# PABannier/bark.cpp

Measured on AMD Instinct MI355X. Metric: audio-sec/sec (RTF), bark-small f16 greedy, higher is better.
Workload: dtype f16 (f32 accumulate); 1 GPU; BASELINE config 2: bark-small f16 on 1xMI355X, single prompt per step, greedy, hipGraph decode, n_steps_text_encoder=256

## Files before the change

bark.cpp_amd/api.py:

```python
from __future__ import annotations

import ctypes as C
import math
import os
import subprocess

import numpy as np

_HERE = os.path.dirname(os.path.abspath(__file__))

PROGRESS_CB = C.CFUNCTYPE(None, C.c_void_p, C.c_int, C.c_int, C.c_void_p)


class BarkContextParams(C.Structure):
    _fields_ = [
        ("verbosity", C.c_int), ("temp", C.c_float), ("fine_temp", C.c_float), ("min_eos_p", C.c_float),
        ("sliding_window_size", C.c_int32), ("max_coarse_history", C.c_int32), ("sample_rate", C.c_int32),
        ("target_bandwidth", C.c_int32), ("cls_token_id", C.c_int32), ("sep_token_id", C.c_int32),
        ("n_steps_text_encoder", C.c_int32), ("text_pad_token", C.c_int32), ("text_encoding_offset", C.c_int32),
        ("semantic_rate_hz", C.c_float), ("semantic_pad_token", C.c_int32), ("semantic_vocab_size", C.c_int32),
        ("semantic_infer_token", C.c_int32), ("coarse_rate_hz", C.c_float), ("coarse_infer_token", C.c_int32),
        ("coarse_semantic_pad_token", C.c_int32), ("n_coarse_codebooks", C.c_int32), ("n_fine_codebooks", C.c_int32),
        ("codebook_size", C.c_int32), ("progress_callback", PROGRESS_CB), ("progress_callback_user_data", C.c_void_p),
    ]
# ... 9 lines not shown

class BarkHipVoicePrompt(C.Structure):
    _fields_ = [("semantic", C.c_void_p), ("n_semantic", C.c_int32), ("coarse_Tx2", C.c_void_p), ("n_coarse_frames", C.c_int32),
                ("fine_Tx8", C.c_void_p), ("n_fine_frames", C.c_int32)]


class BarkHipAudioFormat(C.Structure):
    _fields_ = [("sample_rate", C.c_int32), ("sample_format", C.c_int32)]


class BarkHipJoinParams(C.Structure):
    _fields_ = [("gap_samples", C.c_int32), ("fade_samples", C.c_int32), ("trim_threshold", C.c_float), ("trim_pad_frames", C.c_int32)]


class BarkHipLongParams(C.Structure):
    _fields_ = [("max_tokens", C.c_int32), ("chain", C.c_int32), ("join", BarkHipJoinParams)]


def join_params(gap_samples: int = 6000, fade_samples: int = 0, trim_threshold: float = 0.0, trim_pad_frames: int = 0) -> BarkHipJoinParams:
    return BarkHipJoinParams(int(gap_samples), int(fade_samples), float(trim_threshold), int(trim_pad_frames))


SPLIT_MAX_CHUNKS = 64
SAMPLE_F32, SAMPLE_S16, SAMPLE_MULAW = 0, 1, 2
SAMPLE_FORMATS = {"f32": SAMPLE_F32, "s16": SAMPLE_S16, "mulaw": SAMPLE_MULAW}
SAMPLE_DTYPES = {SAMPLE_F32: np.float32, SAMPLE_S16: np.int16, SAMPLE_MULAW: np.uint8}


def audio_format(rate: int = 24000, fmt="f32") -> BarkHipAudioFormat:
    return BarkHipAudioFormat(int(rate), SAMPLE_FORMATS[fmt] if isinstance(fmt, str) else int(fmt))


def speed_permille(speed) -> int:
    return int(math.floor(1000.0 * float(speed) + 0.5))


def _voice_struct(voice):
    sem = np.ascontiguousarray(voice.semantic, dtype=np.int32).reshape(-1)
    co = np.ascontiguousarray(voice.coarse, dtype=np.int32).reshape(-1, 2)
    fi = np.ascontiguousarray(voice.fine, dtype=np.int32).reshape(-1, 8)
    return BarkHipVoicePrompt(sem.ctypes.data, len(sem), co.ctypes.data, len(co), fi.ctypes.data, len(fi)), (sem, co, fi)


class BarkHipStats(C.Structure):
    _fields_ = [
        ("t_load_us", C.c_int64), ("t_eval_us", C.c_int64), ("t_semantic_us", C.c_int64), ("t_coarse_us", C.c_int64),
        ("t_fine_us", C.c_int64), ("t_codec_us", C.c_int64), ("n_sample_semantic", C.c_int64), ("n_sample_coarse", C.c_int64),
        ("n_sample_fine", C.c_int64), ("n_semantic", C.c_int32), ("n_frames", C.c_int32), ("n_samples", C.c_int32),
        ("n_near_tie", C.c_int32), ("graph_replays", C.c_int32), ("n_prefix_rows_reused", C.c_int32),
    ]

    def as_dict(self):
        return {k: getattr(self, k) for k, _ in self._fields_}


def library_path() -> str:
    return os.environ.get("BARK_HIP_LIBRARY") or os.path.join(_HERE, "lib", "libbark.so")


def build_library(force: bool = False) -> str:
    if force:
        subprocess.check_call(["rm", "-rf", os.path.join(_HERE, "lib", "obj")])
    subprocess.check_call([os.path.join(_HERE, "build.sh")])
    return library_path()


_LIB = None
VOICE_AUDIO_MAX_SAMPLES = 480000

EXPORTS = [
    "bark_context_default_params", "bark_load_model", "bark_generate_audio", "bark_get_audio_data", "bark_get_audio_data_size",
    "bark_get_load_time", "bark_get_eval_time", "bark_reset_statistics", "bark_model_quantize", "bark_free",
    "ggml_time_init", "ggml_time_us", "ggml_time_ms", "ggml_init", "ggml_free",
    "bark_hip_hparams", "bark_hip_set_params", "bark_hip_tokenize", "bark_hip_bert_tokenize", "bark_hip_gpt_eval",
    "bark_hip_fine_eval", "bark_hip_semantic", "bark_hip_coarse", "bark_hip_fine", "bark_hip_fine_many", "bark_hip_codec_decode", "bark_hip_codec_tap",
    "bark_hip_clone_context", "bark_hip_generate_audio_batch", "bark_hip_generate_batch", "bark_hip_generate_batch_seeded", "bark_hip_generate_batch_ex", "bark_hip_reserve_batch", "bark_hip_profile_lock_step", "bark_hip_batch_audio", "bark_hip_batch_tokens", "bark_hip_get_semantic_tokens", "bark_hip_get_coarse_tokens", "bark_hip_get_fine_tokens", "bark_hip_get_stats",
    "bark_hip_time_decode_step", "bark_hip_time_gemv", "bark_hip_time_slots", "bark_hip_time_fine_pass", "bark_hip_time_fine_passes", "bark_hip_describe", "bark_hip_set_fine_order", "bark_hip_load_model_on_device", "bark_hip_batcher_create_multi",
    "bark_hip_batcher_create", "bark_hip_batcher_create_ex", "bark_hip_batcher_submit", "bark_hip_batcher_submit_ex", "bark_hip_batcher_wait", "bark_hip_batcher_stats", "bark_hip_batcher_admitted", "bark_hip_batcher_free",
    "bark_hip_set_sampling_filter", "bark_hip_generate_batch_filtered", "bark_hip_batcher_submit_filtered", "bark_hip_sample_rows_filtered", "bark_hip_time_sample_filter",
    "bark_hip_set_voice_prompt", "bark_hip_generate_batch_voiced", "bark_hip_batcher_submit_voiced", "bark_hip_pick_rows",
    "bark_hip_has_codec_encoder", "bark_hip_codec_encode", "bark_hip_codec_encode_many", "bark_hip_codec_encode_tap", "bark_hip_rvq_encode", "bark_hip_codec_encode_latents", "bark_hip_codec_encode_device_us",
    "bark_hip_load_semantic_encoder", "bark_hip_has_semantic_encoder", "bark_hip_semantic_encode", "bark_hip_semantic_encode_tap", "bark_hip_semantic_head", "bark_hip_semantic_encode_device_us",
    "bark_hip_resample_taps", "bark_hip_resample_24k_to_16k", "bark_hip_voice_from_audio", "bark_hip_set_voice_from_audio", "bark_hip_time_resample",
    "bark_hip_batch_lock_steps",
    "bark_hip_resample_out_len", "bark_hip_resample_table", "bark_hip_resample", "bark_hip_resample_many", "bark_hip_get_audio_as", "bark_hip_batch_audio_as",
    "bark_hip_batcher_submit_as", "bark_hip_batcher_wait_bytes", "bark_hip_time_resample_pair",
    "bark_hip_split_text", "bark_hip_generate_long", "bark_hip_long_audio_as", "bark_hip_long_chunks", "bark_hip_long_chunk_audio", "bark_hip_long_chunk_tokens",
    "bark_hip_join_many", "bark_hip_time_join", "bark_hip_batcher_submit_long", "bark_hip_batcher_ticket_chunks", "bark_hip_time_join_activity",
    "bark_hip_tempo_out_len", "bark_hip_tempo_window", "bark_hip_tempo", "bark_hip_tempo_many", "bark_hip_tempo_positions", "bark_hip_get_audio_at",
    "bark_hip_batch_audio_at", "bark_hip_long_audio_at", "bark_hip_batcher_submit_at", "bark_hip_batcher_submit_long_at", "bark_hip_time_tempo",
]


def load_library() -> C.CDLL:
    global _LIB
    if _LIB is not None:
        return _LIB
    path = library_path()
    if not os.path.exists(path):
        raise RuntimeError(f"{path} is missing - run bark.cpp_amd/build.sh (there is no fallback path)")
    lib = C.CDLL(path)
    vp, ip, fp = C.c_void_p, C.c_void_p, C.c_void_p
    lib.bark_context_default_params.restype = BarkContextParams
    lib.bark_context_default_params.argtypes = []
    lib.bark_load_model.restype = vp
    lib.bark_load_model.argtypes = [C.c_char_p, BarkContextParams, C.c_uint32]
    lib.bark_generate_audio.restype = C.c_bool
    lib.bark_generate_audio.argtypes = [vp, C.c_char_p, C.c_int]
    lib.bark_get_audio_data.restype = C.POINTER(C.c_float)
    lib.bark_get_audio_data.argtypes = [vp]
    lib.bark_get_audio_data_size.restype = C.c_int
    lib.bark_get_audio_data_size.argtypes = [vp]
    lib.bark_get_load_time.restype = C.c_int64
    lib.bark_get_load_time.argtypes = [vp]
    lib.bark_get_eval_time.restype = C.c_int64
    lib.bark_get_eval_time.argtypes = [vp]
    lib.bark_reset_statistics.argtypes = [vp]
    lib.bark_model_quantize.restype = C.c_bool
    lib.bark_model_quantize.argtypes = [C.c_char_p, C.c_char_p, C.c_int]
    lib.bark_free.argtypes = [vp]
    lib.ggml_time_us.restype = C.c_int64
    lib.bark_hip_hparams.argtypes = [vp, C.c_int, ip]
    lib.bark_hip_set_params.argtypes = [vp, BarkContextParams]
    lib.bark_hip_tokenize.argtypes = [vp, C.c_char_p, ip]
    lib.bark_hip_bert_tokenize.argtypes = [vp, C.c_char_p, ip, C.c_int]
    lib.bark_hip_gpt_eval.argtypes = [vp, C.c_int, ip, C.c_int, C.c_int, C.c_int, fp]
    lib.bark_hip_fine_eval.argtypes = [vp, ip, C.c_int, fp]
    lib.bark_hip_semantic.argtypes = [vp, ip, ip, C.c_int, fp]
    lib.bark_hip_coarse.argtypes = [vp, ip, C.c_int, ip, C.c_int]
    lib.bark_hip_fine.argtypes = [vp, ip, C.c_int, ip, C.c_int]
    lib.bark_hip_fine_many.argtypes = [vp, ip, ip, C.c_int, ip, C.c_int]
    lib.bark_hip_codec_decode.argtypes = [vp, ip, C.c_int, C.c_int, fp, C.c_int]
    lib.bark_hip_codec_tap.argtypes = [vp, ip, C.c_int, C.c_int, C.c_int, fp, C.c_int]
    lib.bark_hip_has_codec_encoder.argtypes = [vp]
    lib.bark_hip_codec_encode.argtypes = [vp, fp, C.c_int, C.c_int, ip, C.c_int]
    lib.bark_hip_codec_encode_many.argtypes = [vp, C.POINTER(C.c_void_p), ip, C.c_int, C.c_int, ip, C.c_int]
    lib.bark_hip_codec_encode_tap.argtypes = [vp, fp, C.c_int, C.c_int, fp, C.c_int]
    lib.bark_hip_rvq_encode.argtypes = [vp, fp, C.c_int, C.c_int, ip]
    lib.bark_hip_codec_encode_latents.argtypes = [vp, fp, C.c_int]
    lib.bark_hip_codec_encode_device_us.restype = C.c_double
    lib.bark_hip_codec_encode_device_us.argtypes = [vp]
    lib.bark_hip_load_semantic_encoder.argtypes = [vp, C.c_char_p]
    lib.bark_hip_has_semantic_encoder.argtypes = [vp]
    lib.bark_hip_semantic_encode.argtypes = [vp, fp, C.c_int, ip, C.c_int]
    lib.bark_hip_semantic_encode_tap.argtypes = [vp, fp, C.c_int, C.c_int, fp, C.c_int]
    lib.bark_hip_semantic_head.argtypes = [vp, fp, C.c_int, ip, fp]
    lib.bark_hip_semantic_encode_device_us.restype = C.c_double
    lib.bark_hip_semantic_encode_device_us.argtypes = [vp]
    lib.bark_hip_resample_taps.argtypes = [fp]
    lib.bark_hip_resample_24k_to_16k.argtypes = [vp, fp, C.c_int, fp, C.c_int]
    lib.bark_hip_voice_from_audio.argtypes = [vp, fp, C.c_int, ip, C.c_int, ip, ip, C.c_int, ip, ip]
    lib.bark_hip_set_voice_from_audio.argtypes = [vp, fp, C.c_int]
    lib.bark_hip_time_resample.restype = C.c_double
    lib.bark_hip_time_resample.argtypes = [vp, C.c_int, C.c_int]
    lib.bark_hip_resample_out_len.argtypes = [C.c_int, C.c_int, C.c_int]
    lib.bark_hip_resample_table.argtypes = [C.c_int, C.c_int, fp, C.c_int, ip]
    lib.bark_hip_resample.argtypes = [vp, fp, C.c_int, C.c_int, C.c_int, fp, C.c_int]
    lib.bark_hip_resample_many.argtypes = [vp, C.POINTER(C.c_void_p), ip, C.c_int, C.c_int, C.POINTER(BarkHipAudioFormat), vp, C.c_int, ip]
    lib.bark_hip_get_audio_as.argtypes = [vp, C.POINTER(BarkHipAudioFormat), vp, C.c_int]
    lib.bark_hip_batch_audio_as.argtypes = [vp, C.c_int, C.POINTER(BarkHipAudioFormat), vp, C.c_int]
    lib.bark_hip_time_resample_pair.restype = C.c_double
    lib.bark_hip_time_resample_pair.argtypes = [vp, C.c_int, C.c_int, C.c_int, C.c_int, C.c_int]
    lib.bark_hip_batcher_submit_as.restype = C.c_int64
    lib.bark_hip_batcher_submit_as.argtypes = [vp, C.c_char_p, C.POINTER(BarkHipRequestParams), C.POINTER(BarkHipSamplingFilter), C.POINTER(BarkHipVoicePrompt),
                                               C.POINTER(BarkHipAudioFormat)]
    lib.bark_hip_batcher_wait_bytes.argtypes = [vp, C.c_int64, vp, C.c_int]
    lib.bark_hip_batcher_submit_long.restype = C.c_int64
    lib.bark_hip_batcher_submit_long.argtypes = [vp, C.c_char_p, C.POINTER(BarkHipLongParams), C.POINTER(BarkHipRequestParams), C.POINTER(BarkHipSamplingFilter),
                                                 C.POINTER(BarkHipVoicePrompt), C.POINTER(BarkHipAudioFormat)]
    lib.bark_hip_batcher_ticket_chunks.argtypes = [vp, C.c_int64]
    lib.bark_hip_time_join_activity.restype = C.c_double
    lib.bark_hip_time_join_activity.argtypes = [vp, C.c_int, C.c_int, C.c_int]
    lib.bark_hip_split_text.argtypes = [vp, C.c_char_p, C.c_int, ip, C.c_int]
    lib.bark_hip_generate_long.argtypes = [vp, C.c_char_p, C.POINTER(BarkHipLongParams), C.POINTER(BarkHipRequestParams), C.POINTER(BarkHipSamplingFilter),
                                           C.POINTER(BarkHipVoicePrompt)]
    lib.bark_hip_long_audio_as.argtypes = [vp, C.POINTER(BarkHipAudioFormat), vp, C.c_int]
    lib.bark_hip_long_chunks.argtypes = [vp, ip, C.c_int]
    lib.bark_hip_long_chunk_audio.argtypes = [vp, C.c_int, C.POINTER(C.POINTER(C.c_float))]
    lib.bark_hip_long_chunk_tokens.argtypes = [vp, C.c_int, C.c_int, ip, C.c_int]
    lib.bark_hip_join_many.argtypes = [vp, C.POINTER(C.c_void_p), ip, C.c_int, C.POINTER(BarkHipJoinParams), C.POINTER(BarkHipAudioFormat), vp, C.c_int, ip]
    lib.bark_hip_tempo_out_len.argtypes = [C.c_int, C.c_int]
    lib.bark_hip_tempo_window.argtypes = [fp]
    lib.bark_hip_tempo.argtypes = [vp, fp, C.c_int, C.c_int, fp, C.c_int]
    lib.bark_hip_tempo_many.argtypes = [vp, C.POINTER(C.c_void_p), ip, C.c_int, ip, C.POINTER(BarkHipAudioFormat), vp, C.c_int, ip]
    lib.bark_hip_tempo_positions.argtypes = [vp, fp, C.c_int, C.c_int, ip, C.c_int]
    lib.bark_hip_get_audio_at.argtypes = [vp, C.POINTER(BarkHipAudioFormat), C.c_int, vp, C.c_int]
    lib.bark_hip_batch_audio_at.argtypes = [vp, C.c_int, C.POINTER(BarkHipAudioFormat), C.c_int, vp, C.c_int]
    lib.bark_hip_long_audio_at.argtypes = [vp, C.POINTER(BarkHipAudioFormat), C.c_int, vp, C.c_int]
    lib.bark_hip_batcher_submit_at.restype = C.c_int64
    lib.bark_hip_batcher_submit_at.argtypes = [vp, C.c_char_p, C.POINTER(BarkHipRequestParams), C.POINTER(BarkHipSamplingFilter), C.POINTER(BarkHipVoicePrompt),
                                               C.POINTER(BarkHipAudioFormat), C.c_int]
    lib.bark_hip_batcher_submit_long_at.restype = C.c_int64
    lib.bark_hip_batcher_submit_long_at.argtypes = [vp, C.c_char_p, C.POINTER(BarkHipLongParams), C.POINTER(BarkHipRequestParams), C.POINTER(BarkHipSamplingFilter),
                                                    C.POINTER(BarkHipVoicePrompt), C.POINTER(BarkHipAudioFormat), C.c_int]
    lib.bark_hip_time_tempo.restype = C.c_double
    lib.bark_hip_time_tempo.argtypes = [vp, C.c_int, C.c_int, C.c_int, C.c_int]
    lib.bark_hip_time_join.restype = C.c_double
    lib.bark_hip_time_join.argtypes = [vp, C.c_int, C.c_int, C.c_int, C.c_int, C.c_int]
    lib.bark_hip_generate_batch.argtypes = [vp, C.POINTER(C.c_char_p), C.c_int]
    lib.bark_hip_generate_batch_seeded.argtypes = [vp, C.POINTER(C.c_char_p), C.c_int, C.POINTER(C.c_uint32)]
    lib.bark_hip_generate_batch_ex.argtypes = [vp, C.POINTER(C.c_char_p), C.c_int, C.POINTER(BarkHipRequestParams)]
    lib.bark_hip_reserve_batch.argtypes = [vp, C.c_int]
    lib.bark_hip_set_fine_order.argtypes = [vp, C.c_int]
    lib.bark_hip_profile_lock_step.argtypes = [vp, C.c_int, C.c_int, C.c_int, C.c_int, C.c_char_p, C.c_int]
    lib.bark_hip_batch_audio.argtypes = [vp, C.c_int, C.POINTER(C.POINTER(C.c_float))]
    lib.bark_hip_batch_tokens.argtypes = [vp, C.c_int, C.c_int, ip, C.c_int]
    lib.bark_hip_batch_lock_steps.restype = C.c_int
    lib.bark_hip_batch_lock_steps.argtypes = [vp, C.POINTER(C.c_int32)]
    lib.bark_hip_clone_context.restype = vp
    lib.bark_hip_clone_context.argtypes = [vp, C.c_uint32]
    lib.bark_hip_generate_audio_batch.argtypes = [C.POINTER(C.c_void_p), C.POINTER(C.c_char_p), C.c_int]
    lib.bark_hip_get_semantic_tokens.argtypes = [vp, ip, C.c_int]
    lib.bark_hip_get_coarse_tokens.argtypes = [vp, ip, C.c_int]
    lib.bark_hip_get_fine_tokens.argtypes = [vp, ip, C.c_int]
    lib.bark_hip_get_stats.argtypes = [vp, C.POINTER(BarkHipStats)]
    lib.bark_hip_time_decode_step.restype = C.c_double
    lib.bark_hip_time_decode_step.argtypes = [vp, C.c_int, C.c_int, C.c_int, C.POINTER(C.c_double)]
    lib.bark_hip_time_gemv.restype = C.c_double
    lib.bark_hip_time_gemv.argtypes = [vp, C.c_int, C.c_int, C.c_int, C.POINTER(C.c_double)]
    lib.bark_hip_time_slots.restype = C.c_double
    lib.bark_hip_time_slots.argtypes = [vp, C.c_int, C.c_int, C.c_int, C.c_int, C.c_int, C.c_int]
    lib.bark_hip_time_fine_pass.restype = C.c_double
    lib.bark_hip_time_fine_pass.argtypes = [vp, C.c_int, C.POINTER(C.c_double)]
    lib.bark_hip_batcher_create.restype = vp
    lib.bark_hip_batcher_create.argtypes = [vp, C.c_int, C.c_int]
    lib.bark_hip_batcher_create_ex.restype = vp
    lib.bark_hip_batcher_create_ex.argtypes = [vp, C.c_int, C.c_int, C.c_int]
    lib.bark_hip_load_model_on_device.restype = vp
    lib.bark_hip_load_model_on_device.argtypes = [C.c_char_p, BarkContextParams, C.c_uint32, C.c_int]
    lib.bark_hip_batcher_create_multi.restype = vp
    lib.bark_hip_batcher_create_multi.argtypes = [C.POINTER(C.c_void_p), C.c_int, C.c_int, C.c_int]
    lib.bark_hip_batcher_submit.restype = C.c_int64
    lib.bark_hip_batcher_submit.argtypes = [vp, C.c_char_p, C.c_uint32]
    lib.bark_hip_batcher_submit_ex.restype = C.c_int64
    lib.bark_hip_batcher_submit_ex.argtypes = [vp, C.c_char_p, C.POINTER(BarkHipRequestParams)]
    lib.bark_hip_batcher_submit_filtered.restype = C.c_int64
    lib.bark_hip_batcher_submit_filtered.argtypes = [vp, C.c_char_p, C.POINTER(BarkHipRequestParams), C.POINTER(BarkHipSamplingFilter)]
    lib.bark_hip_set_sampling_filter.argtypes = [vp, C.c_int32, C.c_float]
    lib.bark_hip_generate_batch_filtered.argtypes = [vp, C.POINTER(C.c_char_p), C.c_int, C.POINTER(BarkHipRequestParams), C.POINTER(BarkHipSamplingFilter)]
    lib.bark_hip_sample_rows_filtered.argtypes = [vp, fp, C.c_int, C.c_int, fp, fp, fp, fp, fp, fp]
    lib.bark_hip_time_sample_filter.restype = C.c_double
    lib.bark_hip_time_sample_filter.argtypes = [vp, C.c_int, C.c_int, C.c_int32, C.c_float, C.c_int, C.c_int]
    lib.bark_hip_set_voice_prompt.argtypes = [vp, C.POINTER(BarkHipVoicePrompt)]
    lib.bark_hip_generate_batch_voiced.argtypes = [vp, C.POINTER(C.c_char_p), C.c_int, C.POINTER(BarkHipRequestParams), C.POINTER(BarkHipSamplingFilter),
                                                   C.POINTER(C.POINTER(BarkHipVoicePrompt))]
    lib.bark_hip_batcher_submit_voiced.restype = C.c_int64
    lib.bark_hip_batcher_submit_voiced.argtypes = [vp, C.c_char_p, C.POINTER(BarkHipRequestParams), C.POINTER(BarkHipSamplingFilter), C.POINTER(BarkHipVoicePrompt)]
    lib.bark_hip_pick_rows.argtypes = [vp, fp, C.c_int, C.c_int, C.c_float, fp, ip, ip, ip]
    lib.bark_hip_batcher_wait.argtypes = [vp, C.c_int64, fp, C.c_int]
    lib.bark_hip_batcher_stats.restype = None
    lib.bark_hip_batcher_stats.argtypes = [vp, C.POINTER(C.c_int), C.POINTER(C.c_int), C.POINTER(C.c_int)]
    lib.bark_hip_batcher_admitted.argtypes = [vp]
    lib.bark_hip_batcher_free.restype = None
    lib.bark_hip_batcher_free.argtypes = [vp]
    lib.bark_hip_time_fine_passes.restype = C.c_double
    lib.bark_hip_time_fine_passes.argtypes = [vp, C.c_int, C.c_int, C.POINTER(C.c_double)]
    lib.bark_hip_describe.restype = C.c_char_p
    lib.bark_hip_describe.argtypes = [vp]
    _LIB = lib
    return lib


def default_params(**overrides) -> BarkContextParams:
    p = load_library().bark_context_default_params()
    for k, v in overrides.items():
        setattr(p, k, v)
    return p


def _i32(a):
    return np.ascontiguousarray(a, dtype=np.int32)


class BarkContext:

    def __init__(self, handle, lib):
        self._h = handle
        self._lib = lib
        self._cb = None
        self._params = None

    @classmethod
    def load_model(cls, model_path: str, params: BarkContextParams | None = None, seed: int = 0, device: int | None = None) -> "BarkContext":
        lib = load_library()
        params = params if params is not None else default_params()
        if device is None:
            h = lib.bark_load_model(os.fsencode(model_path), params, seed)
        else:
            h = lib.bark_hip_load_model_on_device(os.fsencode(model_path), params, seed, int(device))
        if not h:
            raise RuntimeError(f"bark_load_model failed for {model_path}")
# ... 774 lines not shown
```

bark.cpp_amd/csrc/api.hip:

```cpp
#include "engine.h"

#include <algorithm>
#include <chrono>
#include <cstdio>
#include <cstring>
#include <stdexcept>
#include <thread>
#include <vector>

using namespace barkhip;

#define HIP_OK_API(expr) do { if ((expr) != hipSuccess) throw std::runtime_error("HIP error at " #expr); } while (0)

namespace {
int64_t wall_us() {
    return std::chrono::duration_cast<std::chrono::microseconds>(std::chrono::steady_clock::now().time_since_epoch()).count();
}
template <typename F> auto guarded(const char * what, decltype(std::declval<F>()()) fail, F && f, bool uses_gpu = true) -> decltype(f()) {
    try {
        if (!uses_gpu) return f();
        (void) hipGetLastError();
        auto r = f();
        const hipError_t e = hipGetLastError();
        if (e != hipSuccess) { fprintf(stderr, "%s: a kernel launch failed: %s\n", what, hipGetErrorString(e)); return fail; }
        return r;
    }
    catch (const std::exception & e) { fprintf(stderr, "%s: %s\n", what, e.what()); }
    catch (...) { fprintf(stderr, "%s: unknown failure\n", what); }
    return fail;
}
}

extern "C" {

struct bark_context_params bark_context_default_params(void) {
    struct bark_context_params p;
    memset(&p, 0, sizeof(p));
    p.verbosity = LOW;
    p.temp = 0.7f;
    p.fine_temp = 0.5f;
    p.min_eos_p = 0.2f;
    p.sliding_window_size = 60;
    p.max_coarse_history = 630;
    p.sample_rate = 24000;
    p.target_bandwidth = 6;
    p.cls_token_id = 101;
    p.sep_token_id = 102;
    p.n_steps_text_encoder = 768;
    p.text_pad_token = 129595;
    p.text_encoding_offset = 10048;
    p.semantic_rate_hz = 49.9f;
    p.semantic_pad_token = 10000;
    p.semantic_vocab_size = 10000;
    p.semantic_infer_token = 129599;
    p.coarse_rate_hz = 75.0f;
    p.coarse_infer_token = 12050;
    p.coarse_semantic_pad_token = 12048;
    p.n_coarse_codebooks = 2;
    p.n_fine_codebooks = 8;
    p.codebook_size = 1024;
    p.progress_callback = nullptr;
    p.progress_callback_user_data = nullptr;
    return p;
}

struct bark_context * bark_load_model(const char * model_path, struct bark_context_params params, uint32_t seed) {
    const int64_t t0 = wall_us();
    if (!model_path) { fprintf(stderr, "bark_load_model: null path\n"); return nullptr; }
    bark_context * ctx = guarded("bark_load_model", (bark_context *) nullptr, [&] { return engine_load(model_path, params, seed); });
    if (ctx) ctx->stats.t_load_us = wall_us() - t0;
    return ctx;
}

bool bark_generate_audio(struct bark_context * bctx, const char * text, int n_threads) {
    (void) n_threads;
    if (!bctx || !text) { fprintf(stderr, "bark_generate_audio: null argument\n"); return false; }
    return guarded("bark_generate_audio", false, [&] { return engine_generate(bctx, text); });
}

float * bark_get_audio_data(struct bark_context * bctx) { return (bctx && !bctx->audio.empty()) ? bctx->audio.data() : nullptr; }
int bark_get_audio_data_size(struct bark_context * bctx) { return bctx ? (int) bctx->audio.size() : 0; }
int64_t bark_get_load_time(struct bark_context * bctx) { return bctx ? bctx->stats.t_load_us : 0; }
int64_t bark_get_eval_time(struct bark_context * bctx) { return bctx ? bctx->stats.t_eval_us : 0; }
// ... 665 lines not shown
}
int bark_hip_set_sampling_filter(struct bark_context * bctx, int32_t top_k, float top_p) {
    const bark_hip_sampling_filter f{top_k, top_p};
    if (!bctx || !filter_valid(f)) return -1;
    return guarded("bark_hip_set_sampling_filter", -1, [&] {
        if (filter_on(f) != filter_on(bctx->filter)) engine_invalidate_graphs(bctx);
        bctx->filter = f;
        return 0;
    });
}
int bark_hip_set_voice_prompt(struct bark_context * bctx, const struct bark_hip_voice_prompt * voice) {
    if (!bctx) return -1;
    return guarded("bark_hip_set_voice_prompt", -1, [&] {
        VoicePtr v = engine_make_voice(bctx, voice);
        bctx->voice = v;
        return 0;
    }, false);
}
int bark_hip_generate_batch_voiced(struct bark_context * bctx, const char * const * texts, int n, const struct bark_hip_request_params * per_utterance,
                                   const struct bark_hip_sampling_filter * filters, const struct bark_hip_voice_prompt * const * voices) {
    if (!bctx || !texts || n <= 0) return -1;
    for (int i = 0; i < n; i++) if (!texts[i]) return -1;
    if (filters) for (int i = 0; i < n; i++) if (!filter_valid(filters[i])) return -1;
    return guarded("bark_hip_generate_batch_voiced", -1, [&] {
        std::vector<VoicePtr> vs;
        if (voices) for (int i = 0; i < n; i++) vs.push_back(engine_make_voice(bctx, voices[i]));
        return engine_generate_batch(bctx, texts, n, nullptr, per_utterance, nullptr, filters, voices ? vs.data() : nullptr);
    });
}
int bark_hip_pick_rows(struct bark_context * bctx, const float * logits, int n_windows, int n_cols, float temp, const double * u, const int32_t * rel,
                       int32_t * tokens_io, int32_t * near_ties) {
    if (!bctx || !logits || !rel || !tokens_io) return -1;
    return guarded("bark_hip_pick_rows", -1, [&] { engine_pick_rows(bctx, logits, n_windows, n_cols, temp, u, rel, tokens_io, near_ties); return 0; });
}
int bark_hip_sample_rows_filtered(struct bark_context * bctx, const float * logits, int n_rows, int n, const float * temp, const int32_t * top_k,
                                  const float * top_p, const double * u, int32_t * out_ids, float * out_eos_p) {
    if (!bctx || !logits || !temp || !top_k || !top_p || !u || !out_ids || n_rows <= 0) return -1;
    return guarded("bark_hip_sample_rows_filtered", -1, [&] { engine_sample_rows_filtered(bctx, logits, n_rows, n, temp, top_k, top_p, u, out_ids, out_eos_p); return 0; });
}
double bark_hip_time_sample_filter(struct bark_context * bctx, int n, int n_slots, int32_t top_k, float top_p, int peaked, int iters) {
    if (!bctx) return -1.0;
    return guarded("bark_hip_time_sample_filter", -1.0, [&] { return engine_time_sample_filtered(bctx, n, n_slots, top_k, top_p, peaked, iters); });
}
int bark_hip_profile_lock_step(struct bark_context * bctx, int which, int n_slots, int ctx, int reps, char * json_out, int capacity) {
    if (!bctx || !json_out || capacity < 2) return -1;
    return guarded("bark_hip_profile_lock_step", -1, [&] {
        std::vector<std::pair<std::string, double>> tl;
        engine_profile_lock_step(bctx, which, n_slots, ctx, reps, tl);
        std::string js = "[";
        for (size_t i = 0; i < tl.size(); i++) {
            char buf[160];
            snprintf(buf, sizeof(buf), "%s{\"site\": \"%s\", \"us\": %.3f}", i ? ", " : "", tl[i].first.c_str(), tl[i].second);
            js += buf;
        }
        js += "]";
        if ((int) js.size() + 1 > capacity) return -1;
        memcpy(json_out, js.c_str(), js.size() + 1);
        return (int) js.size();
    });
}
int bark_hip_reserve_batch(struct bark_context * bctx, int slots) {
    if (!bctx) return -1;
    return guarded("bark_hip_reserve_batch", -1, [&] { engine_reserve_batch(bctx, slots); return 0; });
}
int bark_hip_batch_audio(struct bark_context * bctx, int i, float ** data) {
    if (!bctx || i < 0 || i >= (int) bctx->batch_results.size() || !bctx->batch_results[(size_t) i].ok) return -1;
    if (data) *data = bctx->batch_results[(size_t) i].audio.data();
    return (int) bctx->batch_results[(size_t) i].audio.size();
}
int bark_hip_batch_tokens(struct bark_context * bctx, int i, int stage, int32_t * out, int capacity) {
    if (!bctx || i < 0 || i >= (int) bctx->batch_results.size() || stage < 0 || stage > 2) return -1;
    const auto & r = bctx->batch_results[(size_t) i];
    const std::vector<int32_t> & v = stage == 0 ? r.semantic : stage == 1 ? r.coarse : r.fine;
    if (!out || capacity < (int) v.size()) return -1;
    if (!v.empty()) memcpy(out, v.data(), v.size() * 4);
    return (int) v.size();
}
int bark_hip_batch_lock_steps(struct bark_context * bctx, int32_t out2[2]) {
    if (!bctx || !out2 || bctx->job_lock_steps[0] < 0) return -1;
    out2[0] = bctx->job_lock_steps[0]; out2[1] = bctx->job_lock_steps[1];
    return 0;
}

static int copy_out(const std::vector<int32_t> & v, int per_row, int32_t * out, int capacity_rows) {
    const int rows = (int) v.size() / per_row;
    if (!out || capacity_rows < rows) return -1;
    if (rows) memcpy(out, v.data(), v.size() * 4);
    return rows;
}
int bark_hip_get_semantic_tokens(struct bark_context * bctx, int32_t * out, int capacity) { return bctx ? copy_out(bctx->semantic_tokens, 1, out, capacity) : -1; }
int bark_hip_get_coarse_tokens(struct bark_context * bctx, int32_t * out, int capacity_rows) { return bctx ? copy_out(bctx->coarse_tokens, 2, out, capacity_rows) : -1; }
int bark_hip_get_fine_tokens(struct bark_context * bctx, int32_t * out, int capacity_rows) { return bctx ? copy_out(bctx->fine_tokens, 8, out, capacity_rows) : -1; }

void bark_hip_get_stats(struct bark_context * bctx, struct bark_hip_stats * out) { if (bctx && out) *out = bctx->stats; }

double bark_hip_time_decode_step(struct bark_context * bctx, int which, int ctx, int iters, double * bytes_per_step) {
    if (!bctx) return -1.0;
    return guarded("bark_hip_time_decode_step", -1.0, [&] { return engine_time_decode_step(bctx, which, ctx, iters, bytes_per_step); });
}
double bark_hip_time_gemv(struct bark_context * bctx, int which, int op, int iters, double * bytes_per_launch) {
    if (!bctx) return -1.0;
    return guarded("bark_hip_time_gemv", -1.0, [&] { return engine_time_gemv(bctx, which, op, iters, bytes_per_launch); });
}
double bark_hip_time_fine_passes(struct bark_context * bctx, int n_windows, int iters, double * flops_per_pass) {
    if (!bctx) return -1.0;
    return guarded("bark_hip_time_fine_passes", -1.0, [&] { return engine_time_fine_pass(bctx, iters, flops_per_pass, n_windows); });
}

double bark_hip_time_fine_pass(struct bark_context * bctx, int iters, double * flops_per_pass) {
    if (!bctx) return -1.0;
    return guarded("bark_hip_time_fine_pass", -1.0, [&] { return engine_time_fine_pass(bctx, iters, flops_per_pass); });
}
double bark_hip_time_slots(struct bark_context * bctx, int which, int op, int n_slots, int kind, int ctx, int iters) {
    if (!bctx) return -1.0;
    return guarded("bark_hip_time_slots", -1.0, [&] { return engine_time_slots(bctx, which, op, n_slots, kind, ctx, iters); });
}
#ifdef BARK_TRACE
__attribute__((visibility("default"))) int bark_hip_trace_decode_step(struct bark_context * bctx, int which, int ctx, int replays, unsigned long long * out6, int cap_records) {
    if (!bctx || !out6) return -1;
    return guarded("bark_hip_trace_decode_step", -1, [&] { return engine_trace_decode_step(bctx, which, ctx, replays, out6, cap_records); });
}
#endif
const char * bark_hip_describe(struct bark_context * bctx) { return bctx ? bctx->description.c_str() : "no context"; }

}
```

bark.cpp_amd/csrc/engine.h:

```cpp
#pragma once
#include "bark.h"
#include "bark_mi355x.h"
#include "kernels.h"
#include "model_file.h"
#include "tokenizer.h"

#include <functional>
#include <map>
#include <memory>
#include <random>
#include <string>
#include <vector>

struct bark_context;

namespace barkhip {

struct GraphExec {
    GraphExec() = default;
    explicit GraphExec(hipGraphExec_t exec) : e(exec) {}
    GraphExec(GraphExec && o) noexcept : e(o.e) { o.e = nullptr; }
    GraphExec & operator=(GraphExec && o) noexcept { if (this != &o) { reset(); e = o.e; o.e = nullptr; } return *this; }
    ~GraphExec() { reset(); }
    void reset() { if (e) (void) hipGraphExecDestroy(e); e = nullptr; }
    explicit operator bool() const { return e != nullptr; }
    hipGraphExec_t get() const { return e; }
private:
    hipGraphExec_t e = nullptr;
};
struct Event {
    Event() = default;
    Event(Event && o) noexcept : e(o.e) { o.e = nullptr; }
    Event & operator=(Event && o) noexcept { if (this != &o) { reset(); e = o.e; o.e = nullptr; } return *this; }
    ~Event() { reset(); }
    void reset() { if (e) (void) hipEventDestroy(e); e = nullptr; }
    void record(hipStream_t s);
    hipEvent_t get() const { return e; }
private:
    hipEvent_t e = nullptr;
};
template <typename T> struct DevBuf {
    T * p = nullptr; size_t n = 0;
    void reserve(bark_context * ctx, size_t count);
};

struct GptModel {
    GptHparams hp;
    const half_t * wte[8] = {};
    const half_t * lm_head[8] = {};
    bool q4 = false;
    bool w32 = false;
    QMat wte_q[8], lm_head_q[8];
    const float * wpe = nullptr, * lnf_g = nullptr, * lnf_b = nullptr;
    struct Layer {
        const float * ln1_g = nullptr, * ln1_b = nullptr, * ln2_g = nullptr, * ln2_b = nullptr;
        const half_t * attn_w = nullptr, * proj_w = nullptr, * fc_w = nullptr, * mproj_w = nullptr;
        QMat attn_q, proj_q, fc_q, mproj_q;
        const float * attn_b = nullptr, * proj_b = nullptr, * fc_b = nullptr, * mproj_b = nullptr;
    };
    std::vector<Layer> layers;
    size_t kv_layer_stride = 0;
};
struct GptRun {
    float * kcache = nullptr, * vcache = nullptr;
    float * vtcache = nullptr;
    GraphExec decode_graph[5];
    GraphExec decode_graph8[5];
    GraphExec bench_graph;
};

struct CodecModel {
    CodecHparams hp;
    int n_q = 0, D = 0;
    const float * codebooks = nullptr;
    struct Conv { const half_t * w = nullptr; const float * w32 = nullptr; const float * b = nullptr; const half_t * wm = nullptr; int cout = 0, cin = 0, k = 0; };
    struct ConvT { const half_t * w = nullptr; const float * w32 = nullptr; const float * b = nullptr; const half_t * wm = nullptr; int cin = 0, cout = 0, k = 0, stride = 0; };
    struct Lstm { const half_t * w_ih = nullptr, * w_hh = nullptr; const float * b_ih = nullptr, * b_hh = nullptr; };
    Conv init, fin;
    Lstm lstm[2];
    struct Block { ConvT up; Conv c1, c2, sc; } blocks[4];
    struct EncBlock { Conv c1, c2, sc, down; int stride = 0; };
    struct Encoder { bool present = false; int F = 0; Conv init, fin; EncBlock blocks[4]; Lstm lstm[2]; } enc;
};

struct HubertModel {
    HubertHparams hp;
    int device = 0;
    std::vector<void *> bufs;
    const half_t * conv0_w = nullptr; const float * gn_g = nullptr, * gn_b = nullptr; int k0 = 0;
    struct Conv { const half_t * wm = nullptr; const float * w32 = nullptr; int k = 0, stride = 0; } conv[6];
    const float * fp_ln_g = nullptr, * fp_ln_b = nullptr, * fp_b = nullptr; const half_t * fp_w = nullptr;
    const half_t * pos_w = nullptr; const float * pos_b = nullptr; int pos_co32 = 0, pos_kd = 0, pos_kd16 = 0;
    const float * enc_ln_g = nullptr, * enc_ln_b = nullptr;
    struct Layer {
        const half_t * qkv_w = nullptr, * o_w = nullptr, * fc1_w = nullptr, * fc2_w = nullptr;
        const float * qkv_b = nullptr, * o_b = nullptr, * fc1_b = nullptr, * fc2_b = nullptr, * ln1_g = nullptr, * ln1_b = nullptr, * ln2_g = nullptr, * ln2_b = nullptr;
    };
    std::vector<Layer> layers;
    CodecModel::Lstm lstm[2];
    const half_t * out_w = nullptr; const float * out_b = nullptr;
    const uint16_t * gelu_erf_lut = nullptr;
    HubertModel() = default;
    HubertModel(const HubertModel &) = delete;
    HubertModel & operator=(const HubertModel &) = delete;
    ~HubertModel();
};
constexpr int kHubMaxFrames = 1024;

struct VoicePrompt { std::vector<int32_t> semantic, coarse, fine; };
using VoicePtr = std::shared_ptr<const VoicePrompt>;

}

struct bark_context_memory {
    int device = 0;
    hipStream_t stream = nullptr;
    std::vector<void *> allocs;
    std::vector<void *> pinned;
    bark_context_memory() = default;
    bark_context_memory(const bark_context_memory &) = delete;
    bark_context_memory & operator=(const bark_context_memory &) = delete;
    ~bark_context_memory();
};

struct bark_context : bark_context_memory {
    struct SharedWeights { void * slab = nullptr; void * codebooks = nullptr; std::vector<void *> extra; int device = 0; ~SharedWeights(); };
    std::shared_ptr<SharedWeights> weights;
    std::shared_ptr<const barkhip::HubertModel> hub;

    bark_context_params params;
    std::mt19937 rng;

    barkhip::Vocab vocab;
    barkhip::GptModel gpt[3];
    barkhip::GptRun gpt_run[3];
    barkhip::CodecModel codec;
    bool use_graph = true;
    int fine_order = 0;
    bool in_job = false;
    int fast_gemm = 0;
    int decode_ng = 4;

    size_t weight_bytes = 0;
    std::vector<std::pair<void *, size_t>> guarded;
    float * x = nullptr, * q = nullptr, * logits = nullptr;
    float * knew = nullptr;
    float * ps = nullptr;
    barkhip::half_t * xn = nullptr, * att = nullptr, * hbuf = nullptr;
    barkhip::half_t * q16 = nullptr, * k16 = nullptr, * vt16 = nullptr;
    bool any_q4 = false;
    float * att32 = nullptr, * h32 = nullptr; barkhip::Q8Scratch xq;
    bool any_w32 = false; float * xn32 = nullptr;
    int32_t * d_tokens = nullptr, * d_out_tokens = nullptr;
    float * d_eos_trace = nullptr;
    barkhip::StepState * d_state = nullptr;
    double * d_u = nullptr;
    bool host_sampling = false;
    bark_hip_sampling_filter filter{0, 1.0f};
    int32_t * d_filter = nullptr;
    barkhip::VoicePtr voice;
    int32_t * d_fine_rel = nullptr;
    uint16_t * d_gelu_lut = nullptr;
    int max_E = 0, max_H = 0, P = 1024;
    barkhip::DevBuf<float> cbuf[3];
    barkhip::DevBuf<barkhip::half_t> cbuf_hh[3];
    barkhip::DevBuf<float> c_gi, c_cell, c_cell2; barkhip::DevBuf<barkhip::half_t> c_hseq_h, c_xt_h, c_hseq2_h;
    barkhip::DevBuf<int32_t> d_codes;
    barkhip::GraphExec fine_graphs[16];
    int * d_lstm_t = nullptr;
    barkhip::DevBuf<int> d_codec_T;
    struct LstmGraph { barkhip::GraphExec exec; int B = 0; const float * out = nullptr; const float * gi = nullptr; } lstm_graph;
    LstmGraph lstm_graph_enc;
    barkhip::DevBuf<int> d_enc_T;
    barkhip::DevBuf<float> d_pcm;
    barkhip::Event enc_ev[2]; double enc_device_us = -1.0;
    const float * enc_latents = nullptr; int enc_latent_rows = 0;
    LstmGraph lstm_graph_hub;
    struct HubScratch {
        bool ready = false;
        float * pcm = nullptr; barkhip::half_t * pcm_h = nullptr;
        barkhip::half_t * a16 = nullptr, * b16 = nullptr;
        double * part = nullptr; float * stats = nullptr;
        float * feat = nullptr;
        float * x = nullptr, * tmp = nullptr, * q = nullptr, * kc = nullptr, * vc = nullptr;
        barkhip::half_t * xh = nullptr, * att = nullptr, * hb = nullptr;
        float * gi = nullptr, * c1 = nullptr, * c2 = nullptr, * out2 = nullptr; barkhip::half_t * h1 = nullptr, * h2 = nullptr;
        float * logits = nullptr; int32_t * ids = nullptr;
        int * rows = nullptr;
        barkhip::DevBuf<float> tap;
    } hubs;
    barkhip::Event hub_ev[2]; double hub_device_us = -1.0;
    barkhip::DevBuf<float> rs_in, rs_out;
    std::map<std::pair<int, int>, const float *> rp_taps;
    barkhip::DevBuf<float> rp_in; barkhip::DevBuf<uint8_t> rp_out; barkhip::DevBuf<int> rp_seg;
    barkhip::DevBuf<int> jn_tab; barkhip::DevBuf<float> jn_fade; int jn_fade_F = -1;
    barkhip::DevBuf<float> tp_in, tp_out, tp_win; barkhip::DevBuf<int> tp_seg, tp_pos; bool tp_win_ready = false;
    struct CodecGraph { barkhip::GraphExec exec; std::vector<int> T; const float * buf = nullptr; float * out = nullptr; int tmul = 0; } codec_graph;

    struct Batch {
        int cap = 0;
        float * kc[2] = {nullptr, nullptr}, * vc[2] = {nullptr, nullptr}; size_t slot_stride[2] = {0, 0};
        float * x = nullptr, * q = nullptr, * logits = nullptr; barkhip::half_t * att = nullptr, * h = nullptr;
        barkhip::StepState * state = nullptr; int32_t * out_tokens = nullptr; float * eos_trace = nullptr; float * ln_stats = nullptr;
        float * att32 = nullptr, * h32 = nullptr;
        float * sc = nullptr;
        float * ps = nullptr;
        double * u = nullptr;
        size_t ld_logits = 0;
        float * slot_par = nullptr;
        int32_t * slot_top_k = nullptr;
        int32_t * h_ids = nullptr; barkhip::StepState * h_state = nullptr, * h_state_in = nullptr;
        float * pf_x = nullptr, * pf_q = nullptr; barkhip::half_t * pf_xn = nullptr, * pf_att = nullptr, * pf_h = nullptr;
        int32_t * pf_tokens = nullptr; barkhip::SeqTab * pf_tab = nullptr;
    } batch;
    std::vector<float> h_slot_par;
    std::vector<int32_t> h_slot_top_k;
    struct StepMark { std::string name; barkhip::Event at; };
    std::vector<StepMark> * step_marks = nullptr;
    std::map<int, barkhip::GraphExec> batch_graphs;
    struct FineBatch {
        int cap = 0;
        float * x = nullptr, * q = nullptr, * logits = nullptr, * kc = nullptr, * vc = nullptr;
        barkhip::half_t * xn = nullptr, * att = nullptr, * hbuf = nullptr, * q16 = nullptr, * k16 = nullptr, * vt16 = nullptr;
        int32_t * tokens = nullptr, * rel = nullptr;
        double * u = nullptr;
    } fine_batch;
    struct BatchResult { std::vector<int32_t> semantic, coarse, fine; std::vector<float> audio; bool ok = false; };
    std::vector<BatchResult> batch_results;
    struct LongResult {
        std::vector<barkhip::TextSpan> spans; std::vector<BatchResult> chunks; bark_hip_join_params join{6000, 0, 0.0f, 0};
        std::vector<uint8_t> joined; std::vector<int32_t> layout; bark_hip_audio_format joined_fmt{0, 0};
        int joined_speed = 1000;
    } long_result;
    int32_t job_lock_steps[2] = {-1, -1};
    bark_context * tail = nullptr;

#ifdef BARK_TRACE
    unsigned long long * trace_rec = nullptr; unsigned * trace_pos = nullptr; unsigned trace_cap = 0; int trace_kid = 0; unsigned trace_base = 0, trace_per_replay = 0;
// ... 83 lines not shown
```

bark.cpp_amd/csrc/engine.hip:

```cpp
#include "engine_internal.h"

#include <algorithm>
#include <climits>
#include <cmath>
#include <cstdio>
#include <cstdlib>
#include <cstring>
#include <deque>
#include <stdexcept>

using namespace barkhip;
using namespace barkhip::detail;

namespace barkhip {

namespace detail {

double weight_bytes_per_element(const GptModel & m) {
    if (m.w32) return 4.0;
    if (m.q4) return quant_formats()[m.layers[0].attn_q.qt].block_bytes / 32.0;
    return 2.0;
}

bool fine_products_on_f16_mfma(const bark_context * c, const GptModel & m, bool causal) {
// ... 51 lines not shown
        if (!kbase && !vbase) a.vt = layer_vt(c, m, l);
        a.seq = seq; a.kv_slot_stride = kv_seq_stride; a.seqtab = seqtab;
        if (flash) {
            a.epi = EPI_QKV16; a.q16 = rb.q16; a.k16 = rb.k16; a.vt16 = rb.vt16; a.seq = 1024;
            launch_linear(s, a);
            AttnFlashArgs fa;
            fa.q16 = rb.q16; fa.k16 = rb.k16; fa.vt16 = rb.vt16; fa.H = H; fa.E = E; fa.S = 1024; fa.Z = N / 1024; fa.att = rb.att; fa.ld_att = E;
            launch_attn_flash(s, fa);
        } else {
            launch_linear(s, a);
            AttnPrefillArgs at;
            at.q = rb.q; at.ldq = E; at.kc = layer_k(m, l); at.vc = layer_v(m, l); at.H = H; at.P = P; at.N = seq > 0 ? seq : N; at.n_past = pos0;
            at.causal = causal ? 1 : 0; at.att = rb.att; at.ld_att = E; at.att32 = m.q4 ? c->att32 : nullptr;
            at.Z = Z; at.kv_seq_stride = kv_seq_stride; at.seqtab = seqtab;
            launch_attn_prefill(s, at);
        }
        if (m.q4 && !m.w32) launch_q8_rows(s, c->att32, N, E, nullptr, nullptr, c->xq);
        LinArgs p = layer_product(c, m, l, OP_PROJ);
        rows_in(p, rb.att, c->att32);
        p.res = rb.x;
        launch_linear(s, p);
        LinArgs f = layer_product(c, m, l, OP_FC);
        ln_rows(f);
        rows_in(f, rb.xn, c->xn32);
        f.out_h = rb.hbuf; f.out_h32 = m.q4 ? c->h32 : nullptr;
        launch_linear(s, f);
        if (m.q4 && !m.w32) launch_q8_rows(s, c->h32, N, 4 * E, nullptr, nullptr, c->xq);
        LinArgs o = layer_product(c, m, l, OP_MPROJ);
        rows_in(o, rb.hbuf, c->h32);
        o.res = rb.x;
        launch_linear(s, o);
    }
}

void run_layers_decode(bark_context * c, GptModel & m) {
    const int E = m.hp.n_embd, H = m.hp.n_head, P = c->P;
    hipStream_t s = c->stream;
    for (int l = 0; l < m.hp.n_layer; l++) {
        const bool ps = !(crosscheck_mask() & 4) && !m.w32 && P == 1024 && run_of(c, m).vtcache && E <= 1024;
        LinArgs a = layer_product(c, m, l, OP_QKV);
        a.x_f32 = c->x; a.q = c->q; a.kc = layer_k(c, m, l); a.vc = layer_v(c, m, l); a.vt = layer_vt(c, m, l); a.st = c->d_state;
        if (ps) { a.ps = c->ps; a.knew = c->knew; a.ng = c->decode_ng; }
        BARK_TRACE_SET(c, a, (a.M + 3) / 4 + 4 * (E / 4));
        launch_linear(s, a);
        AttnDecodeArgs at;
        at.q = c->q; at.kc = layer_k(c, m, l); at.vc = layer_v(c, m, l); at.H = H; at.P = P; at.st = c->d_state; at.att = c->att;
        at.att32 = m.q4 ? c->att32 : nullptr;
        if (ps) { at.ps = c->ps; at.knew = c->knew; at.ng = c->decode_ng; at.vt = layer_vt(c, m, l); }
        BARK_TRACE_SET(c, at, 8 * 16 * ((H + 7) / 8) * 16);
        launch_attn_decode(s, at);
        LinArgs p = layer_product(c, m, l, OP_PROJ);
        if (m.q4) p.x_f32 = c->att32; else p.x_f16 = c->att;
        p.res = c->x;
        BARK_TRACE_SET(c, p, (p.M + 3) / 4);
        launch_linear(s, p);
        LinArgs f = layer_product(c, m, l, OP_FC);
        f.x_f32 = c->x; f.out_h = c->hbuf; f.out_h32 = m.q4 ? c->h32 : nullptr;
        BARK_TRACE_SET(c, f, (f.M + 3) / 4);
        launch_linear(s, f);
        LinArgs o = layer_product(c, m, l, OP_MPROJ);
        if (m.q4) o.x_f32 = c->h32; else o.x_f16 = c->hbuf;
        o.res = c->x;
        BARK_TRACE_SET(c, o, (o.M + 3) / 4);
        launch_linear(s, o);
    }
}

LinArgs lm_head_args(const GptModel & m, int row0, int n_rows, int parity_rows, const float * xrow, float * out, int ld_out, const StepState * st) {
    const int E = m.hp.n_embd;
    LinArgs a;
    if (m.q4) a.wq = q4_rows(m.lm_head_q[0], (size_t) row0, E); else a.W = m.lm_head[0] + (size_t) row0 * E;
    a.M = n_rows; a.K = E; a.N = 1;
    a.x_f32 = xrow; a.ln_g = m.lnf_g; a.ln_b = m.lnf_b; a.epi = EPI_LOGITS; a.out = out; a.ld_out = ld_out;
    a.parity_rows = parity_rows; a.st = st;
    return a;
}
void run_lm_head(bark_context * c, GptModel & m, const float * xrow, int row0, int n_rows, int parity_rows, float out_div) {
    LinArgs a = lm_head_args(m, row0, n_rows, parity_rows, xrow, c->logits, n_rows, c->d_state);
    a.out_div = out_div;
    BARK_TRACE_SET(c, a, (a.M + 3) / 4);
    launch_linear(c->stream, a);
}

void set_state(bark_context * c, const StepState & st) {
    HIP_OK(hipMemcpyAsync(c->d_state, &st, sizeof(st), hipMemcpyHostToDevice, c->stream));
    HIP_OK(hipStreamSynchronize(c->stream));
}
StepState get_state(bark_context * c) {
    StepState st;
    HIP_OK(hipMemcpyAsync(&st, c->d_state, sizeof(st), hipMemcpyDeviceToHost, c->stream));
    HIP_OK(hipStreamSynchronize(c->stream));
    if (st.fault) throw std::runtime_error("decode step launched with a context bound below the cached keys (partial scores incomplete)");
    return st;
}
StepState fresh_state() {
    StepState st{};
    st.eos_step = INT32_MAX;
    return st;
}

void upload_tokens(bark_context * c, const int32_t * tok, size_t n) {
    HIP_OK(hipMemcpyAsync(c->d_tokens, tok, n * 4, hipMemcpyHostToDevice, c->stream));
    HIP_OK(hipStreamSynchronize(c->stream));
}

void check_ids(const int32_t * tok, size_t n, int n_in, const char * what) {
    for (size_t i = 0; i < n; i++)
        if (tok[i] < 0 || tok[i] >= n_in) throw std::runtime_error(std::string(what) + ": token id out of range");
}

int run_prefill(bark_context * c, GptModel & m, int n_tokens, bool merge, float * kbase, float * vbase, int pos0) {
    const int N = merge ? n_tokens - 256 : n_tokens;
    EmbedArgs e;
    set_token_embedding(e, c, m);
    e.tokens = c->d_tokens; e.n_rows = N; e.merge = merge ? 1 : 0; e.pos0 = pos0; e.x = c->x;
    launch_embed_causal(c->stream, e);
    run_layers_rows(c, m, N, true, kbase, vbase, pos0);
    return N;
}

StageCfg stage_cfg(bark_context * c, int which) {
    const bark_context_params & p = c->params;
    StageCfg s{};
    s.which = which;
    s.temp = p.temp;
    if (which == 0) {
        s.mode = 0; s.lm_row0 = 0; s.lm_rows = c->gpt[0].hp.n_out_vocab; s.parity_rows = 0; s.token_base = 0;
        s.min_eos_p = p.min_eos_p; s.eos_token = p.semantic_vocab_size;
    } else {
        s.mode = 1; s.lm_row0 = p.semantic_vocab_size; s.lm_rows = p.codebook_size; s.parity_rows = p.codebook_size;
        s.token_base = p.semantic_vocab_size; s.min_eos_p = 0.f; s.eos_token = -1;
    }
    return s;
}

void embed_state_row(bark_context * c, const GptModel & m, const StepState * st, float * x) {
    EmbedArgs e;
    set_token_embedding(e, c, m);
    e.n_rows = 1; e.st = st; e.x = x;
    launch_embed_causal(c->stream, e);
}

void run_sample(bark_context * c, const StageCfg & s, int n_past_add, bool prescaled) {
    SampleArgs a;
    a.prescaled = prescaled ? 1 : 0;
    a.logits = c->logits; a.n = s.lm_rows; a.mode = s.mode; a.min_eos_p = s.min_eos_p; a.eos_token = s.eos_token;
    a.token_base = s.token_base; a.n_past_add = n_past_add; a.out_tokens = c->d_out_tokens;
    a.eos_trace = s.mode == 0 ? c->d_eos_trace : nullptr; a.st = c->d_state;
    a.temp = s.temp; a.u = c->d_u;
    a.force_exact = exact_sampling();
    set_token_embedding(a, c, c->gpt[s.which]);
    a.x = c->x;
    BARK_TRACE_SET(c, a, 16);
    if (!prescaled && s.temp > 0.0f && filter_on(c->filter)) launch_sample_filtered(c->stream, a, c->d_filter, reinterpret_cast<const float *>(c->d_filter + 1));
    else launch_sample_greedy(c->stream, a);
}

void enqueue_decode_step(bark_context * c, const StageCfg & s, bool sample, int n_past_add, bool embed) {
    GptModel & m = c->gpt[s.which];
    if (embed) embed_state_row(c, m, c->d_state, c->x);
    run_layers_decode(c, m);
    const bool prescale = sample && s.temp == 0.0f;
    run_lm_head(c, m, c->x, s.lm_row0, s.lm_rows, s.parity_rows, prescale ? 0.7f : 0.0f);
    if (sample) run_sample(c, s, n_past_add, prescale);
}

GraphExec capture_graph(hipStream_t s, const std::function<void()> & body) {
    hipGraph_t graph = nullptr;
    hipGraphExec_t exec = nullptr;
    HIP_OK(hipStreamBeginCapture(s, hipStreamCaptureModeThreadLocal));
    try { body(); }
    catch (...) { hipGraph_t g2 = nullptr; (void) hipStreamEndCapture(s, &g2); if (g2) (void) hipGraphDestroy(g2); throw; }
    HIP_OK(hipStreamEndCapture(s, &graph));
    const hipError_t err = hipGraphInstantiate(&exec, graph, nullptr, nullptr, 0);
    (void) hipGraphDestroy(graph);
    HIP_OK(err);
    return GraphExec(exec);
}

double time_on_stream_us(bark_context * c, const std::function<void()> & body) {
    Event e0, e1;
    e0.record(c->stream);
    body();
    e1.record(c->stream);
    HIP_OK(hipEventSynchronize(e1.get()));
    float ms = 0.f;
    HIP_OK(hipEventElapsedTime(&ms, e0.get(), e1.get()));
    return (double) ms * 1000.0;
}

GraphExec capture_decode(bark_context * c, const StageCfg & s, int n_past_add, int n_steps, int ng) {
    struct Restore { bark_context * c; int ng; ~Restore() { c->decode_ng = ng; } } restore{c, c->decode_ng};
    c->decode_ng = std::max(1, std::min(ng, 4));
    return capture_graph(c->stream, [&] { for (int i = 0; i < n_steps; i++) enqueue_decode_step(c, s, true, n_past_add, false); });
}

void decode_steps_greedy(bark_context * c, const StageCfg & s, int n, int n_past) {
    GptRun & run = c->gpt_run[s.which];
    if (!c->use_graph) {
        struct Restore { bark_context * c; ~Restore() { c->decode_ng = 4; } } restore{c};
        for (int k = 0; k < n; k++) { c->decode_ng = std::min(4, (n_past + k + 256) / 256); enqueue_decode_step(c, s, true, 1, false); }
        return;
    }
    int k = 0;
    while (k < n) {
        const int g = n - k >= 8 ? 8 : 1;
        const int ng = std::min(4, (n_past + k + g + 255) / 256);
        GraphExec & e = g == 8 ? run.decode_graph8[ng] : run.decode_graph[ng];
        if (!e) e = capture_decode(c, s, 1, g, ng);
        HIP_OK(hipGraphLaunch(e.get(), c->stream));
        c->stats.graph_replays++;
        k += g;
    }
}

void filter_host(std::vector<float> & l, int32_t top_k, float top_p) {
    const int n = (int) l.size();
    if (n == 0 || (top_k <= 0 && !(top_p < 1.0f))) return;
    std::vector<int> ord((size_t) n);
    for (int i = 0; i < n; i++) ord[(size_t) i] = i;
    std::sort(ord.begin(), ord.end(), [&](int a, int b) { return l[(size_t) a] > l[(size_t) b] || (l[(size_t) a] == l[(size_t) b] && a < b); });
    int J = n;
    if (top_p < 1.0f) {
        float mx = -INFINITY;
        for (float v : l) mx = std::max(mx, v);
        std::vector<uint64_t> w((size_t) n);
        uint64_t S = 0;
        for (int i = 0; i < n; i++) { const float e = (float) exp((double) (l[(size_t) i] - mx)); w[(size_t) i] = (uint64_t) std::floor((double) e * 1099511627776.0); S += w[(size_t) i]; }
        int ex = 0; const double fr = std::frexp((double) top_p, &ex);
        const unsigned __int128 fm = (unsigned __int128) std::ldexp(fr, 24);
        const int sh = 24 - ex;
        const unsigned __int128 prod = fm * (unsigned __int128) S;
        const uint64_t T = sh >= 128 ? 0 : (uint64_t) (prod >> sh);
        uint64_t W = 0;
        J = 0;
        for (int j = 0; j < n; j++) {
            if (j > 0 && W > T) break;
            J = j + 1;
            W += w[(size_t) ord[(size_t) j]];
        }
    }
    int F = J;
    if (top_k > 0 && top_k < J) {
        const float v = l[(size_t) ord[(size_t) top_k - 1]];
        F = top_k;
        while (F < J && l[(size_t) ord[(size_t) F]] >= v) F++;
    }
    for (int j = F; j < n; j++) l[(size_t) ord[(size_t) j]] = -INFINITY;
}
void softmax_host(std::vector<float> & l) {
    float mx = -INFINITY;
    for (float v : l) mx = std::max(mx, v);
    float sum = 0.0f;
    for (float & v : l) { v = (float) exp((double) (v - mx)); sum += v; }
    for (float & v : l) v /= sum;
}
int sample_host(std::vector<float> & l, std::mt19937 & rng, float temp, float * eos_p, const bark_hip_sampling_filter * flt) {
    if (temp == 0.0f) {
        for (float & v : l) v /= 0.7f;
        softmax_host(l);
        if (eos_p) *eos_p = l.back();
        int best = 0; float mx = -INFINITY;
        for (int i = 0; i < (int) l.size(); i++) if (l[(size_t) i] > mx) { mx = l[(size_t) i]; best = i; }
        return best;
    }
    if (flt) filter_host(l, flt->top_k, flt->top_p);
    for (float & v : l) v /= temp;
    softmax_host(l);
    std::discrete_distribution<int32_t> dist(l.begin(), l.end());
    const int next = dist(rng);
    if (eos_p) *eos_p = l.back();
    return next;
}

std::vector<float> fetch_logits(bark_context * c, size_t n) {
    std::vector<float> l(n);
    HIP_OK(hipMemcpyAsync(l.data(), c->logits, n * 4, hipMemcpyDeviceToHost, c->stream));
    HIP_OK(hipStreamSynchronize(c->stream));
    return l;
}

void upload_uniforms(bark_context * c, int n) {
    if (n > 8192) throw std::runtime_error("too many samples in one stage");
    std::mt19937 tmp = c->rng;
    std::vector<double> u((size_t) n);
    for (auto & v : u) v = std::generate_canonical<double, 53>(tmp);
    HIP_OK(hipMemcpyAsync(c->d_u, u.data(), (size_t) n * sizeof(double), hipMemcpyHostToDevice, c->stream));
    HIP_OK(hipStreamSynchronize(c->stream));
}
void consume_uniforms(bark_context * c, int n_used) { c->rng.discard(2ull * (unsigned long long) n_used); }
void upload_filter(bark_context * c) {
    int32_t v[2] = {c->filter.top_k, 0};
    memcpy(&v[1], &c->filter.top_p, 4);
    HIP_OK(hipMemcpyAsync(c->d_filter, v, sizeof(v), hipMemcpyHostToDevice, c->stream));
    HIP_OK(hipStreamSynchronize(c->stream));
}

void progress(bark_context * c, bark_encoding_step step, int pct) {
    if (c->params.progress_callback) c->params.progress_callback(c, step, pct, c->params.progress_callback_user_data);
}

}

int engine_gpt_eval(bark_context * c, int which, const int32_t * tokens, int n_tokens, int n_past, bool merge_ctx, float * logits) {
    if (which < 0 || which > 1) throw std::runtime_error("gpt_eval: which must be 0 or 1");
    HIP_OK(hipSetDevice(c->device));
    GptModel & m = c->gpt[which];
    const bool merge = merge_ctx && n_past == 0;
    if (n_tokens <= 0) throw std::runtime_error("gpt_eval: no tokens");
    if (n_past > 0 && n_tokens != 1) throw std::runtime_error("gpt_eval: n_past > 0 needs exactly one token");
    if (merge && n_tokens != 513) throw std::runtime_error("gpt_eval: merged prompt must hold 513 ids");
    const int N = merge ? n_tokens - 256 : n_tokens;
    if (n_past + N > m.hp.block_size) throw std::runtime_error("gpt_eval: context overflow");
    check_ids(tokens, (size_t) n_tokens, m.hp.n_in_vocab, "gpt_eval");
    const int n_out = m.hp.n_out_vocab;
    if (N > 1) {
        upload_tokens(c, tokens, (size_t) n_tokens);
        run_prefill(c, m, n_tokens, merge);
        StepState st = fresh_state();
        set_state(c, st);
        run_lm_head(c, m, c->x + (size_t) (N - 1) * m.hp.n_embd, 0, n_out, 0);
    } else if (n_past == 0) {
        StepState st = fresh_state(); st.n_past = 0; st.cur_token = tokens[0];
        set_state(c, st);
        StageCfg s = stage_cfg(c, which); s.lm_row0 = 0; s.lm_rows = n_out; s.parity_rows = 0;
        enqueue_decode_step(c, s, false, 1);
    } else {
        StepState st = fresh_state(); st.n_past = n_past; st.cur_token = tokens[0];
        set_state(c, st);
        StageCfg s = stage_cfg(c, which); s.lm_row0 = 0; s.lm_rows = n_out; s.parity_rows = 0;
        enqueue_decode_step(c, s, false, 1);
    }
    HIP_OK(hipMemcpyAsync(logits, c->logits, (size_t) n_out * 4, hipMemcpyDeviceToHost, c->stream));
    HIP_OK(hipStreamSynchronize(c->stream));
    return n_past + N;
}

bool filter_valid(const bark_hip_sampling_filter & f) { return f.top_k >= 0 && f.top_p > 0.0f && f.top_p <= 1.0f; }

void engine_sample_rows_filtered(bark_context * c, const float * logits, int n_rows, int n, const float * temp, const int32_t * top_k, const float * top_p,
                                 const double * u, int32_t * out_ids, float * out_eos_p) {
    if (n_rows <= 0 || n < 1 || n > 12288) throw std::runtime_error("sample_rows_filtered: n must be in 1..12288");
    for (int r = 0; r < n_rows; r++)
        if (!(temp[r] >= 0.0f) || !filter_valid(bark_hip_sampling_filter{top_k[r], top_p[r]})) throw std::runtime_error("sample_rows_filtered: bad settings");
    HIP_OK(hipSetDevice(c->device));
    const int chunk = std::min(n_rows, 4096);
    struct Buf { void * p = nullptr; ~Buf() { if (p) (void) hipFree(p); } };
    Buf b_l, b_t, b_k, b_p, b_u, b_st, b_ids, b_eos;
    HIP_OK(hipMalloc(&b_l.p, (size_t) chunk * n * 4)); HIP_OK(hipMalloc(&b_t.p, (size_t) chunk * 4)); HIP_OK(hipMalloc(&b_k.p, (size_t) chunk * 4));
    HIP_OK(hipMalloc(&b_p.p, (size_t) chunk * 4)); HIP_OK(hipMalloc(&b_u.p, (size_t) chunk * 8)); HIP_OK(hipMalloc(&b_st.p, (size_t) chunk * sizeof(StepState)));
    HIP_OK(hipMalloc(&b_ids.p, (size_t) chunk * 4)); HIP_OK(hipMalloc(&b_eos.p, (size_t) chunk * 4));
    std::vector<StepState> sts((size_t) chunk, fresh_state());
    for (int r0 = 0; r0 < n_rows; r0 += chunk) {
        const int nb = std::min(chunk, n_rows - r0);
        hipStream_t st = c->stream;
        HIP_OK(hipMemcpyAsync(b_l.p, logits + (size_t) r0 * n, (size_t) nb * n * 4, hipMemcpyHostToDevice, st));
        HIP_OK(hipMemcpyAsync(b_t.p, temp + r0, (size_t) nb * 4, hipMemcpyHostToDevice, st));
        HIP_OK(hipMemcpyAsync(b_k.p, top_k + r0, (size_t) nb * 4, hipMemcpyHostToDevice, st));
        HIP_OK(hipMemcpyAsync(b_p.p, top_p + r0, (size_t) nb * 4, hipMemcpyHostToDevice, st));
        HIP_OK(hipMemcpyAsync(b_u.p, u + r0, (size_t) nb * 8, hipMemcpyHostToDevice, st));
        HIP_OK(hipMemcpyAsync(b_st.p, sts.data(), (size_t) nb * sizeof(StepState), hipMemcpyHostToDevice, st));
        SampleArgs a;
        a.force_exact = exact_sampling();
        a.logits = (const float *) b_l.p; a.n = n; a.mode = 0; a.eos_token = -1; a.min_eos_p = 2.0f; a.token_base = 0; a.n_past_add = 0;
        a.out_tokens = (int32_t *) b_ids.p; a.eos_trace = (float *) b_eos.p; a.st = (StepState *) b_st.p;
        a.nbatch = nb; a.ld_logits = n; a.out_stride = 1; a.u = (const double *) b_u.p; a.u_stride = 1;
        a.slot_temp = (const float *) b_t.p; a.x = nullptr;
        a.kinds = 0;
        for (int r = r0; r < r0 + nb; r++) {
            a.kinds |= temp[r] > 0.0f ? 2 : 1;
            if (temp[r] > 0.0f && filter_on(bark_hip_sampling_filter{top_k[r], top_p[r]})) a.kinds |= 4;
        }
        launch_sample_filtered(st, a, (const int32_t *) b_k.p, (const float *) b_p.p);
        HIP_OK(hipMemcpyAsync(out_ids + r0, b_ids.p, (size_t) nb * 4, hipMemcpyDeviceToHost, st));
        if (out_eos_p) HIP_OK(hipMemcpyAsync(out_eos_p + r0, b_eos.p, (size_t) nb * 4, hipMemcpyDeviceToHost, st));
        HIP_OK(hipStreamSynchronize(st));
    }
}
// ... 6 lines not shown
    const RowBufs & rb = rbp ? *rbp : own;
    launch_embed_fine(c->stream, m.wte, m.wte_q, m.wpe, E, m.hp.n_in_vocab, rb.tokens, nn, rb.x, N, rb.plane);
    if (rbp) run_layers_rows(c, m, N, false, c->fine_batch.kc, c->fine_batch.vc, 0, rbp, 1024, (size_t) E * c->P);
    else     run_layers_rows(c, m, N, false);
    if (m.w32)     launch_ln_rows_f32(c->stream, rb.x, N, E, m.lnf_g, m.lnf_b, c->xn32);
    else if (m.q4) launch_q8_rows(c->stream, rb.x, N, E, m.lnf_g, m.lnf_b, c->xq);
    else           launch_ln_rows(c->stream, rb.x, N, E, m.lnf_g, m.lnf_b, rb.xn);
    LinArgs a;
    a.W = m.lm_head[nn - 1]; a.wq = m.lm_head_q[nn - 1]; a.xq = c->xq; if (m.w32) a.x_f32 = c->xn32; a.M = n_rows; a.K = E; a.N = N; a.x_f16 = rb.xn; a.epi = EPI_LOGITS; a.out = rb.logits; a.ld_out = n_rows;
    a.fast = fine_products_on_f16_mfma(c, m, false) ? 1 : (!m.q4 && !m.w32) ? c->fast_gemm : 0;
    launch_linear(c->stream, a);
}

FinePlan fine_plan(const bark_context_params & p, const std::vector<int32_t> & coarse, const VoicePrompt * voice) {
    const int nc = p.n_coarse_codebooks, cs = p.codebook_size;
    FinePlan f;
    f.T = (int) coarse.size() / nc;
    if (f.T <= 0 || f.T > 8192) throw std::runtime_error("fine: number of frames must be in 1..8192");
    for (int32_t v : coarse) if (v < 0 || v >= cs) throw std::runtime_error("fine: coarse code out of range");
    const int Tf = voice ? (int) voice->fine.size() / 8 : 0;
    f.n_hist = std::min(Tf, 512);
    f.L = std::max(f.n_hist + f.T, 1024);
    f.in_arr.assign((size_t) f.L * 8, cs);
    for (int t = 0; t < f.n_hist; t++) for (int ch = 0; ch < 8; ch++) f.in_arr[(size_t) t * 8 + ch] = voice->fine[(size_t) (Tf - f.n_hist + t) * 8 + ch];
    for (int t = 0; t < f.T; t++) for (int ch = 0; ch < nc; ch++) f.in_arr[(size_t) (f.n_hist + t) * 8 + ch] = coarse[(size_t) t * nc + ch];
    f.n_loops = std::max(0, (int) ceilf((float) (f.T - (1024 - f.n_hist)) / 512.f)) + 1;
    return f;
}
std::vector<int32_t> fine_plan_result(FinePlan & f) {
    f.in_arr.erase(f.in_arr.begin(), f.in_arr.begin() + (long) f.n_hist * 8);
    f.in_arr.resize((size_t) f.T * 8);
    return std::move(f.in_arr);
}
FineWindow fine_window(const FinePlan & f, int n) {
    FineWindow w;
    w.start_idx = std::min(n * 512, f.L - 1024);
    w.start_fill_idx = std::min(f.n_hist + n * 512, f.L - 512);
    w.rel = w.start_fill_idx - w.start_idx;
    return w;
}
void fine_window_tokens(const FinePlan & f, const FineWindow & w, int32_t * tok, size_t plane) {
    for (int ch = 0; ch < 8; ch++) for (int j = 0; j < 1024; j++) tok[(size_t) ch * plane + j] = f.in_arr[(size_t) (w.start_idx + j) * 8 + ch];
}
void fine_write_back(FinePlan & f, const FineWindow & w, const bark_context_params & p, const int32_t * tok, size_t plane) {
    for (int nn = p.n_coarse_codebooks; nn < p.n_fine_codebooks; nn++)
        for (int j = 0; j < 1024 - w.rel; j++) f.in_arr[(size_t) (w.start_fill_idx + j) * 8 + nn] = tok[(size_t) nn * plane + w.rel + j];
}
}

void engine_fine_eval(bark_context * c, const int32_t * tokens_8x1024, int nn, float * logits) {
    HIP_OK(hipSetDevice(c->device));
    GptModel & m = c->gpt[2];
    if (nn < 1 || nn >= m.hp.n_wtes || nn - 1 >= m.hp.n_lm_heads) throw std::runtime_error("fine_eval: bad codebook index");
    check_ids(tokens_8x1024, 8 * 1024, m.hp.n_in_vocab, "fine_eval");
    upload_tokens(c, tokens_8x1024, 8 * 1024);
    run_fine_forward(c, nn, m.hp.n_out_vocab);
    HIP_OK(hipMemcpyAsync(logits, c->logits, (size_t) 1024 * m.hp.n_out_vocab * 4, hipMemcpyDeviceToHost, c->stream));
    HIP_OK(hipStreamSynchronize(c->stream));
}

std::vector<int32_t> engine_semantic(bark_context * c, const std::vector<int32_t> & prompt, std::vector<float> * eos_trace) {
    HIP_OK(hipSetDevice(c->device));
    const bark_context_params & p = c->params;
    GptModel & m = c->gpt[0];
    if (prompt.size() != 513) throw std::runtime_error("semantic: prompt must hold 513 ids");
    check_ids(prompt.data(), prompt.size(), m.hp.n_in_vocab, "semantic");
    const int n_steps = std::max(0, std::min(p.n_steps_text_encoder, m.hp.block_size - 257 + 1));
    const StageCfg s = stage_cfg(c, 0);
    std::vector<int32_t> out;
    if (n_steps == 0) return out;
    upload_tokens(c, prompt.data(), prompt.size());
    StepState st = fresh_state();
    set_state(c, st);
    const bool greedy = p.temp == 0.0f || !c->host_sampling;
    if (p.temp != 0.0f && greedy) upload_uniforms(c, n_steps);
    if (p.temp != 0.0f && greedy && filter_on(c->filter)) upload_filter(c);
    const int N = run_prefill(c, m, 513, true);
    run_lm_head(c, m, c->x + (size_t) (N - 1) * m.hp.n_embd, s.lm_row0, s.lm_rows, 0);
    if (greedy) {
        run_sample(c, s, N);
        progress(c, SEMANTIC, 100 * 1 / std::max(1, p.n_steps_text_encoder));
        int issued = 1;
        StepState cur{};
        while (true) {
            const int batch_end = std::min(n_steps, issued + 32);
            decode_steps_greedy(c, s, batch_end - issued, N + issued - 1);
            for (; issued < batch_end; issued++) progress(c, SEMANTIC, 100 * (issued + 1) / std::max(1, p.n_steps_text_encoder));
            cur = get_state(c);
            if (cur.eos_step != INT32_MAX || issued >= n_steps) break;
        }
        const int n_keep = std::min(cur.eos_step, issued);
        out.resize((size_t) n_keep);
        if (n_keep) copy_to_host(c, out.data(), c->d_out_tokens, (size_t) n_keep * 4);
        if (eos_trace) {
            const int n_tr = std::min(issued, cur.eos_step == INT32_MAX ? issued : cur.eos_step + 1);
            eos_trace->resize((size_t) n_tr);
            if (n_tr) copy_to_host(c, eos_trace->data(), c->d_eos_trace, (size_t) n_tr * 4);
        }
        const int n_used = std::min(issued, cur.eos_step == INT32_MAX ? issued : cur.eos_step + 1);
        c->stats.n_sample_semantic += n_used;
        c->stats.n_near_tie += cur.near_tie;
        if (p.temp != 0.0f) consume_uniforms(c, n_used);
    } else {
        int n_past = N;
        for (int i = 0; i < n_steps; i++) {
            if (i > 0) {
                StepState h = fresh_state(); h.n_past = n_past; h.cur_token = out.back();
                set_state(c, h);
                enqueue_decode_step(c, s, false, 1);
                n_past += 1;
            }
            std::vector<float> l = fetch_logits(c, (size_t) s.lm_rows);
            float eos_p = 0.f;
            const int next = sample_host(l, c->rng, p.temp, &eos_p, filter_on(c->filter) ? &c->filter : nullptr);
            c->stats.n_sample_semantic++;
            if (eos_trace) eos_trace->push_back(eos_p);
            progress(c, SEMANTIC, 100 * (i + 1) / std::max(1, p.n_steps_text_encoder));
            if (next == p.semantic_vocab_size || eos_p >= p.min_eos_p) break;
            out.push_back(next);
        }
    }
    return out;
}

namespace detail {
VoiceTrim voice_trim(const bark_context_params & p, const VoicePrompt * v) {
    VoiceTrim t;
    if (!v) return t;
    const int nc = p.n_coarse_codebooks;
    const float stc_ratio = p.coarse_rate_hz / p.semantic_rate_hz * nc;
    const int n_sem = (int) v->semantic.size(), n_flat = (int) v->coarse.size();
    const int n_sh = std::min(std::min((int) floorf(p.max_coarse_history / stc_ratio), n_sem - n_sem % 2), (int) floorf(n_flat / stc_ratio));
    const int n_ch = (int) roundf(n_sh * stc_ratio);
    if (n_sh < 2 || n_ch <= 2 || n_ch > n_flat) throw std::runtime_error("voice prompt: the trimmed coarse history is empty");
    t.sem.assign(v->semantic.end() - n_sh, v->semantic.end());
    for (int k = n_flat - n_ch; k < n_flat - 2; k++) t.coarse.push_back(p.semantic_vocab_size + p.codebook_size * (k % nc) + v->coarse[(size_t) k]);
    return t;
}
std::vector<int32_t> coarse_window_prompt(const bark_context_params & p, const VoiceTrim & vt, const std::vector<int32_t> & semantic, const std::vector<int32_t> & out, int step_idx) {
    const float stc_ratio = p.coarse_rate_hz / p.semantic_rate_hz * p.n_coarse_codebooks;
    const int max_semantic_history = (int) floorf(p.max_coarse_history / stc_ratio);
    const int n_sh = (int) vt.sem.size(), n_all = n_sh + (int) semantic.size();
    const int semantic_idx = n_sh + (int) roundf(step_idx / stc_ratio);
    std::vector<int32_t> in;
    in.reserve(257 + (size_t) p.max_coarse_history);
    for (int i = std::max(semantic_idx - max_semantic_history, 0); i < n_all && in.size() < 256; i++) in.push_back(i < n_sh ? vt.sem[(size_t) i] : semantic[(size_t) (i - n_sh)]);
    in.resize(256, p.coarse_semantic_pad_token);
    in.push_back(p.coarse_infer_token);
    const int n_vc = (int) vt.coarse.size(), total = n_vc + (int) out.size();
    for (int k = total - std::min(p.max_coarse_history, total); k < total; k++) in.push_back(k < n_vc ? vt.coarse[(size_t) k] : out[(size_t) (k - n_vc)]);
    return in;
}
}

VoicePtr engine_make_voice(const bark_context * c, const bark_hip_voice_prompt * v) {
    if (!v) return VoicePtr();
    const bark_context_params & p = c->params;
    if (p.n_coarse_codebooks != 2 || p.n_fine_codebooks != 8 || p.codebook_size != 1024) throw std::runtime_error("voice prompt: only 2 -> 8 codebooks of 1024 entries are supported");
    if (v->n_semantic < 0 || v->n_coarse_frames < 0 || v->n_fine_frames < 0 || v->n_semantic > (1 << 20) || v->n_coarse_frames > (1 << 20) || v->n_fine_frames > (1 << 20) ||
        (v->n_semantic && !v->semantic) || (v->n_coarse_frames && !v->coarse_Tx2) || (v->n_fine_frames && !v->fine_Tx8))
        throw std::runtime_error("voice prompt: bad counts or null arrays");
    auto vp = std::make_shared<VoicePrompt>();
    vp->semantic.assign(v->semantic, v->semantic + v->n_semantic);
    vp->coarse.assign(v->coarse_Tx2, v->coarse_Tx2 + (size_t) v->n_coarse_frames * 2);
    vp->fine.assign(v->fine_Tx8, v->fine_Tx8 + (size_t) v->n_fine_frames * 8);
    check_ids(vp->semantic.data(), vp->semantic.size(), p.semantic_vocab_size, "voice prompt (semantic)");
    check_ids(vp->coarse.data(), vp->coarse.size(), p.codebook_size, "voice prompt (coarse)");
    check_ids(vp->fine.data(), vp->fine.size(), p.codebook_size, "voice prompt (fine)");
    const VoiceTrim t = voice_trim(p, vp.get());
    if (p.sliding_window_size > 0 && 257 + std::min(p.max_coarse_history, (int) t.coarse.size()) + p.sliding_window_size - 1 > c->gpt[1].hp.block_size)
        throw std::runtime_error("voice prompt: the history and the first coarse window exceed the coarse model's context");
    return vp;
}
void engine_voice_into_prompt(const bark_context_params & p, const VoicePrompt * v, std::vector<int32_t> & prompt) {
    if (!v || prompt.size() != 513) return;
    const int n = std::min((int) v->semantic.size(), 256);
    for (int i = 0; i < 256; i++) prompt[(size_t) 256 + i] = i < n ? v->semantic[v->semantic.size() - (size_t) n + i] : p.semantic_pad_token;
}

std::vector<int32_t> engine_coarse(bark_context * c, const std::vector<int32_t> & semantic) {
    HIP_OK(hipSetDevice(c->device));
    const bark_context_params & p = c->params;
    GptModel & m = c->gpt[1];
    if (p.n_coarse_codebooks != 2 || p.codebook_size != 1024) throw std::runtime_error("coarse: only 2 codebooks of 1024 entries are supported");
    if (p.sliding_window_size <= 0 || p.max_coarse_history < 0) throw std::runtime_error("coarse: bad window parameters");
    check_ids(semantic.data(), semantic.size(), m.hp.n_in_vocab, "coarse");
    const StageCfg s = stage_cfg(c, 1);
    if (s.lm_row0 + 2 * s.lm_rows > m.hp.n_out_vocab) throw std::runtime_error("coarse: vocabulary too small");
    const float stc_ratio = p.coarse_rate_hz / p.semantic_rate_hz * p.n_coarse_codebooks;
    const int n_steps = (int) (floorf(semantic.size() * stc_ratio / p.n_coarse_codebooks) * p.n_coarse_codebooks);
    if (n_steps <= 0) throw std::runtime_error("coarse: no steps to run");
    const VoiceTrim voice = voice_trim(p, c->voice.get());
    const int n_windows = (int) ceilf((float) n_steps / p.sliding_window_size);
    const bool greedy = p.temp == 0.0f || !c->host_sampling;
    if (p.temp != 0.0f && greedy) upload_uniforms(c, n_steps);
    if (p.temp != 0.0f && greedy && filter_on(c->filter)) upload_filter(c);
    std::vector<int32_t> out;
    std::vector<int32_t> cached;
    const bool reuse_prefix = !(crosscheck_mask() & 8);
    int step_idx = 0;
    for (int w = 0; w < n_windows; w++) {
        const std::vector<int32_t> in = coarse_window_prompt(p, voice, semantic, out, step_idx);
        const int N = (int) in.size();
        const int steps_here = std::min(p.sliding_window_size, n_steps - step_idx);
        if (N + steps_here - 1 > m.hp.block_size)
            throw std::runtime_error(w == 0 && !voice.coarse.empty() ? "coarse: the voice prompt's history and the first window exceed the context" : "coarse: window exceeds the context");
        check_ids(in.data(), in.size(), m.hp.n_in_vocab, "coarse");
        int L = 0;
        if (greedy && reuse_prefix) {
            while (L < N && L < (int) cached.size() && cached[(size_t) L] == in[(size_t) L]) L++;
            if (L >= N) L = N - 1;
        }
        const int rows = N - L;
        StepState st = fresh_state(); st.step = step_idx; st.n_past = L; st.cur_token = in[(size_t) L];
        set_state(c, st);
        if (greedy && rows == 1) {
            embed_state_row(c, m, c->d_state, c->x);
            decode_steps_greedy(c, s, 1, L);
            c->stats.n_prefix_rows_reused += L;
        } else {
            upload_tokens(c, in.data() + L, (size_t) rows);
            run_prefill(c, m, rows, false, nullptr, nullptr, L);
            c->stats.n_prefix_rows_reused += L;
        }
        if (greedy) {
            if (rows > 1) {
                run_lm_head(c, m, c->x + (size_t) (rows - 1) * m.hp.n_embd, s.lm_row0, s.lm_rows, s.parity_rows);
                run_sample(c, s, rows);
            }
            progress(c, COARSE, 100 * (step_idx + 1) / n_steps);
            decode_steps_greedy(c, s, steps_here - 1, N);
            for (int j = 1; j < steps_here; j++) progress(c, COARSE, 100 * (step_idx + j + 1) / n_steps);
            const StepState cur = get_state(c);
            std::vector<int32_t> got((size_t) steps_here);
            copy_to_host(c, got.data(), c->d_out_tokens, (size_t) steps_here * 4);
            out.insert(out.end(), got.begin(), got.end());
            cached = in;
            cached.insert(cached.end(), got.begin(), got.end() - 1);
            step_idx += steps_here;
            c->stats.n_sample_coarse += steps_here;
            c->stats.n_near_tie += cur.near_tie;
        } else {
            int n_past = N;
            for (int j = 0; j < steps_here; j++) {
                const int parity = step_idx % 2;
                if (j == 0) {
                    run_lm_head(c, m, c->x + (size_t) (N - 1) * m.hp.n_embd, s.lm_row0 + parity * s.lm_rows, s.lm_rows, 0);
                } else {
                    StepState h = fresh_state(); h.n_past = n_past; h.cur_token = out.back(); h.step = step_idx;
                    set_state(c, h);
                    StageCfg s2 = s; s2.lm_row0 = s.lm_row0 + parity * s.lm_rows; s2.parity_rows = 0;
                    enqueue_decode_step(c, s2, false, 1);
                    n_past += 1;
                }
                std::vector<float> l = fetch_logits(c, (size_t) s.lm_rows);
                int next = sample_host(l, c->rng, p.temp, nullptr, filter_on(c->filter) ? &c->filter : nullptr);
                next += s.lm_row0 + parity * s.lm_rows;
                out.push_back(next);
                step_idx += 1;
                c->stats.n_sample_coarse++;
                progress(c, COARSE, 100 * step_idx / n_steps);
            }
        }
    }
    if (p.temp != 0.0f && greedy) consume_uniforms(c, n_steps);
    std::vector<int32_t> res;
    for (size_t i = 0; i + 1 < out.size(); i += 2) {
        res.push_back(out[i] - p.semantic_vocab_size);
        res.push_back(out[i + 1] - p.semantic_vocab_size - p.codebook_size);
    }
    return res;
}

std::vector<int32_t> engine_fine(bark_context * c, const std::vector<int32_t> & coarse) {
    HIP_OK(hipSetDevice(c->device));
    const bark_context_params & p = c->params;
    GptModel & m = c->gpt[2];
    const int nc = p.n_coarse_codebooks, nf = p.n_fine_codebooks, cs = p.codebook_size;
    if (nc != 2 || nf != 8 || cs != 1024) throw std::runtime_error("fine: only 2 -> 8 codebooks of 1024 entries are supported");
    FinePlan plan = fine_plan(p, coarse, c->voice.get());
    const int n_loops = plan.n_loops;
    const bool greedy = p.fine_temp == 0.0f;
    const bool device_multinomial = !greedy && !c->host_sampling;
    StepState st = fresh_state();
    set_state(c, st);
    std::vector<int32_t> buf((size_t) 8 * 1024);
    for (int n = 0; n < n_loops; n++) {
        const FineWindow w = fine_window(plan, n);
        const int rel = w.rel;
        fine_window_tokens(plan, w, buf.data(), 1024);
        HIP_OK(hipMemcpyAsync(c->d_fine_rel, &w.rel, 4, hipMemcpyHostToDevice, c->stream));
        upload_tokens(c, buf.data(), buf.size());
        if (device_multinomial) upload_uniforms(c, (nf - nc) * 1024);
        for (int nn = nc; nn < nf; nn++) {
            progress(c, FINE, 100 * (n * (nf - nc) + (nn - nc + 1)) / (n_loops * (nf - nc)));
            if (greedy || device_multinomial) {
                int32_t * pick_dst = c->d_tokens + (size_t) nn * 1024;
                auto enqueue = [&] {
                    run_fine_forward(c, nn, cs);
                    if (greedy) launch_argmax_rows(c->stream, c->logits, cs, 1024, cs, pick_dst, 1, c->d_state, c->d_fine_rel);
                    else launch_sample_rows_multinomial(c->stream, c->logits, cs, 1024, cs, p.fine_temp, c->d_u + (size_t) (nn - nc) * 1024, pick_dst, 1, c->d_state, c->d_fine_rel);
                };
                if (c->use_graph) {
                    GraphExec & g = c->fine_graphs[nn + (fine_products_on_f16_mfma(c, m, false) ? 8 : 0)];
                    if (!g) g = capture_graph(c->stream, enqueue);
                    HIP_OK(hipGraphLaunch(g.get(), c->stream));
                    c->stats.graph_replays++;
                } else {
                    enqueue();
                }
            } else {
                const int n_out = m.hp.n_out_vocab;
                run_fine_forward(c, nn, n_out);
                std::vector<float> l = fetch_logits(c, (size_t) 1024 * n_out);
                std::vector<int32_t> ch(1024);
                for (int i = 0; i < 1024; i++) {
                    std::vector<float> relv(l.begin() + (size_t) i * n_out, l.begin() + (size_t) i * n_out + cs);
                    ch[(size_t) i] = sample_host(relv, c->rng, p.fine_temp, nullptr);
                }
                HIP_OK(hipMemcpyAsync(c->d_tokens + (size_t) nn * 1024 + rel, ch.data() + rel, (size_t) (1024 - rel) * 4, hipMemcpyHostToDevice, c->stream));
                HIP_OK(hipStreamSynchronize(c->stream));
            }
            c->stats.n_sample_fine += 1024;
        }
        if (device_multinomial) consume_uniforms(c, (nf - nc) * 1024);
        HIP_OK(hipMemcpyAsync(buf.data(), c->d_tokens, buf.size() * 4, hipMemcpyDeviceToHost, c->stream));
        HIP_OK(hipStreamSynchronize(c->stream));
        fine_write_back(plan, w, p, buf.data(), 1024);
    }
    const StepState cur = get_state(c);
    c->stats.n_near_tie += cur.near_tie;
    return fine_plan_result(plan);
}

namespace detail {
void ensure_fine_batch(bark_context * c, int Z) {
    bark_context::FineBatch & fb = c->fine_batch;
    if (fb.cap >= Z) return;
    GptModel & m = c->gpt[2];
    const size_t R = (size_t) Z * 1024, E = (size_t) m.hp.n_embd;
    fb.x = dev_alloc<float>(c, R * E); fb.q = dev_alloc<float>(c, R * E);
    fb.xn = dev_alloc<half_t>(c, R * E); fb.att = dev_alloc<half_t>(c, R * E); fb.hbuf = dev_alloc<half_t>(c, R * E * 4);
    fb.kc = dev_alloc<float>(c, (size_t) Z * E * c->P); fb.vc = dev_alloc<float>(c, (size_t) Z * E * c->P);
    if (c->fast_gemm) { fb.q16 = dev_alloc<half_t>(c, R * E); fb.k16 = dev_alloc<half_t>(c, R * E); fb.vt16 = dev_alloc<half_t>(c, R * E); }
    fb.logits = dev_alloc<float>(c, R * 1024);
    fb.tokens = dev_alloc<int32_t>(c, 8 * R); fb.rel = dev_alloc<int32_t>(c, (size_t) Z);
    fb.u = dev_alloc<double>(c, 6 * R);
    fb.cap = Z;
}
RowBufs fine_batch_rows(bark_context * c, int Z) {
    const bark_context::FineBatch & fb = c->fine_batch;
    RowBufs rb; rb.x = fb.x; rb.q = fb.q; rb.xn = fb.xn; rb.att = fb.att; rb.hbuf = fb.hbuf; rb.q16 = fb.q16; rb.k16 = fb.k16; rb.vt16 = fb.vt16;
    rb.logits = fb.logits; rb.tokens = fb.tokens; rb.plane = Z * 1024;
    return rb;
}
}

std::vector<std::vector<int32_t>> engine_fine_many(bark_context * c, const std::vector<const std::vector<int32_t> *> & coarse, std::vector<std::mt19937> * rngs,
                                                   const std::vector<const VoicePrompt *> * voices) {
    HIP_OK(hipSetDevice(c->device));
    const bark_context_params & p = c->params;
    GptModel & m = c->gpt[2];
    const int nc = p.n_coarse_codebooks, nf = p.n_fine_codebooks, cs = p.codebook_size;
    if (nc != 2 || nf != 8 || cs != 1024) throw std::runtime_error("fine: only 2 -> 8 codebooks of 1024 entries are supported");
    if (m.q4 || m.w32 || c->host_sampling) throw std::runtime_error("fine_many: f16 model files, device sampling");
    const JobScope job(c);
    const int U = (int) coarse.size();
    const bool greedy = p.fine_temp == 0.0f;
    if (!greedy && (!rngs || (int) rngs->size() != U)) throw std::runtime_error("fine_many: one generator per utterance is needed for fine_temp > 0");
    if (voices && (int) voices->size() != U) throw std::runtime_error("fine_many: one voice entry per utterance");
    std::vector<FinePlan> us((size_t) U);
    int max_loops = 0;
    for (int u = 0; u < U; u++) {
        us[(size_t) u] = fine_plan(p, *coarse[(size_t) u], voices ? (*voices)[(size_t) u] : c->voice.get());
// ... 129 lines not shown
```

bark.cpp_amd/csrc/engine_codec.hip:

```cpp
#include "engine_internal.h"

#include <algorithm>
#include <cmath>
#include <cstdlib>
#include <cstring>
#include <map>
#include <mutex>
#include <stdexcept>

using namespace barkhip;
using namespace barkhip::detail;


namespace {
void ensure_codec_scratch(bark_context * c, size_t need, int Ts, int D) {
    for (auto & b : c->cbuf) b.reserve(c, need);
    for (auto & b : c->cbuf_hh) b.reserve(c, need);
    const size_t rows = (size_t) Ts * D;
    c->c_gi.reserve(c, 4 * rows); c->c_hseq_h.reserve(c, rows); c->c_xt_h.reserve(c, rows); c->c_hseq2_h.reserve(c, rows);
    c->c_cell.reserve(c, (size_t) 32 * D); c->c_cell2.reserve(c, (size_t) 32 * D); c->d_codec_T.reserve(c, 80);
}

struct LstmIo { const half_t * x_h; int K_in, D; float * gi, * c1, * c2; half_t * h1, * h2; };
LstmIo codec_lstm_io(bark_context * c) { return LstmIo{c->c_xt_h.p, c->codec.D, c->codec.D, c->c_gi.p, c->c_cell.p, c->c_cell2.p, c->c_hseq_h.p, c->c_hseq2_h.p}; }
void run_lstm_pair(bark_context * c, const CodecModel::Lstm * lstm, bark_context::LstmGraph & slot, const CodecBatch & cb, int Ts, int Tmax, float * out2, const LstmIo & io) {
    hipStream_t s = c->stream;
    const int D = io.D, B = cb.B;
    {
        LinArgs g;
        g.W = lstm[0].w_ih; g.M = 4 * D; g.K = io.K_in; g.N = Ts; g.x_f16 = io.x_h; g.epi = EPI_LOGITS; g.out = io.gi; g.ld_out = 4 * D;
        launch_linear(s, g);
    }
    LstmPairArgs a;
    a.gi1 = io.gi; a.w_hh1 = lstm[0].w_hh; a.b_ih1 = lstm[0].b_ih; a.b_hh1 = lstm[0].b_hh; a.c1 = io.c1; a.h1 = io.h1;
    a.w_ih2 = lstm[1].w_ih; a.w_hh2 = lstm[1].w_hh; a.b_ih2 = lstm[1].b_ih; a.b_hh2 = lstm[1].b_hh; a.c2 = io.c2; a.h2 = io.h2;
    a.out2 = out2; a.T = Tmax; a.D = D; a.cb = cb;
    if (!c->use_graph) {
        for (int i = 0; i <= Tmax; i++) { a.t = i; launch_lstm_pair_step(s, a); }
        return;
    }
    constexpr int kBlock = 64;
    if (slot.out != out2 || slot.gi != io.gi || slot.B != B) slot.exec.reset();
    if (!slot.exec) {
        slot.exec = capture_graph(s, [&] {
            a.t_base = c->d_lstm_t;
            for (int i = 0; i < kBlock; i++) { a.t = i; launch_lstm_pair_step(s, a); }
            launch_add_int(s, c->d_lstm_t, kBlock);
        });
        slot.out = out2; slot.gi = io.gi; slot.B = B;
    }
    const int hdr[2] = {0, Tmax};
    HIP_OK(hipMemcpyAsync(c->d_lstm_t, hdr, sizeof(hdr), hipMemcpyHostToDevice, s));
    HIP_OK(hipStreamSynchronize(s));
    for (int i0 = 0; i0 <= Tmax; i0 += kBlock) HIP_OK(hipGraphLaunch(slot.exec.get(), s));
}

void throw_on_missing_pick(const std::vector<int32_t> & codes) {
    for (int32_t v : codes) if (v < 0) throw std::runtime_error("codec: a latent frame has no finite distance to any codebook row (non-finite latent)");
}
}

namespace barkhip {

std::vector<std::vector<float>> engine_codec_decode_many(bark_context * c, const std::vector<const int32_t *> & codes, int n_q, const std::vector<int> & T,
                                                         int tap_stage, std::vector<float> * tap) {
    HIP_OK(hipSetDevice(c->device));
    c->enc_latents = nullptr; c->enc_latent_rows = 0;
    CodecModel & cm = c->codec;
    const int B = (int) T.size();
    if (B < 1 || B > 32 || codes.size() != T.size()) throw std::runtime_error("codec: 1..32 utterances per call");
    if (tap_stage >= 0 && B != 1) throw std::runtime_error("codec: activation taps take one utterance");
    if (n_q <= 0 || n_q > cm.n_q) throw std::runtime_error("codec: bad code matrix shape");
    std::vector<int> Tpre((size_t) B + 1, 0);
    int Tmax = 0;
    for (int b = 0; b < B; b++) {
        if (T[(size_t) b] <= 0 || T[(size_t) b] > 4096) throw std::runtime_error("codec: bad code matrix shape");
        for (size_t i = 0; i < (size_t) n_q * T[(size_t) b]; i++) if (codes[(size_t) b][i] < 0 || codes[(size_t) b][i] >= cm.hp.n_bins) throw std::runtime_error("codec: code out of range");
        Tpre[(size_t) b + 1] = Tpre[(size_t) b] + T[(size_t) b];
        Tmax = std::max(Tmax, T[(size_t) b]);
    }
    const int Ts = Tpre[(size_t) B];
    hipStream_t s = c->stream;
    const int D = cm.D;
    size_t need = (size_t) std::max(cm.hp.hidden_dim, D) * Ts;
    { int ch = D; size_t tt = (size_t) Ts; for (auto & b : cm.blocks) { ch = b.up.cout; tt *= b.up.stride; need = std::max(need, (size_t) ch * tt); } }
    ensure_codec_scratch(c, need, Ts, D);
    c->d_codes.reserve(c, (size_t) n_q * Ts);
    for (int b = 0; b < B; b++)
        HIP_OK(hipMemcpyAsync(c->d_codes.p + (size_t) n_q * Tpre[(size_t) b], codes[(size_t) b], (size_t) n_q * T[(size_t) b] * 4, hipMemcpyHostToDevice, s));
    {
        int hdr[80] = {};
        for (int b = 0; b < B; b++) hdr[b] = T[(size_t) b];
        for (int b = 0; b <= B; b++) hdr[40 + b] = Tpre[(size_t) b];
        HIP_OK(hipMemcpyAsync(c->d_codec_T.p, hdr, sizeof(hdr), hipMemcpyHostToDevice, s));
        HIP_OK(hipStreamSynchronize(s));
    }
    CodecBatch cb; cb.T = c->d_codec_T.p; cb.Tpre = c->d_codec_T.p + 40; cb.B = B;
    float * A = c->cbuf[0].p, * Bf = c->cbuf[1].p, * R = c->cbuf[2].p;
    half_t * H0 = c->cbuf_hh[0].p, * H1 = c->cbuf_hh[1].p, * H2 = c->cbuf_hh[2].p;

    auto conv_args = [&](const half_t * wm, const float * w32, const float * bias, int cin, int cout, int K, int stride, const half_t * xh, int tm_in) {
        ConvTmArgs a;
        a.W = wm; a.w32 = w32; a.bias = bias; a.cin = cin; a.cout = cout; a.cout32 = (cout + 31) & ~31; a.K = K;
        a.convT = stride > 0 ? 1 : 0; a.nphase = stride > 0 ? stride : 1;
        a.kd = (stride > 0 ? 2 : K) * cin; a.kd16 = (a.kd + 15) & ~15;
        a.xh = xh; a.rows_in = Ts * tm_in; a.tm_in = tm_in; a.cb = cb;
        return a;
    };
    auto conv = [&](const CodecModel::Conv & cv, const half_t * xh, int tm, const float * add, float * y, half_t * yh_raw, half_t * yh_elu) {
        ConvTmArgs a = conv_args(cv.wm, cv.w32, cv.b, cv.cin, cv.cout, cv.k, 0, xh, tm);
        a.add = add; a.y = y; a.yh_raw = yh_raw; a.yh_elu = yh_elu;
        launch_conv_tm(s, a);
    };
    launch_rvq_gather(s, cm.codebooks, cm.hp.n_bins, cm.hp.hidden_dim, c->d_codes.p, n_q, Tmax, Ts, A, cb);
    launch_act_round(s, A, (size_t) cm.hp.hidden_dim * Ts, 0, H0);
    conv(cm.init, H0, 1, nullptr, Bf, c->c_xt_h.p, nullptr);
    run_lstm_pair(c, cm.lstm, c->lstm_graph, cb, Ts, Tmax, R, codec_lstm_io(c));
    auto grab = [&](int stage, const float * buf, int C, size_t rows) {
        if (tap_stage != stage || !tap) return;
        std::vector<float> tm((size_t) C * rows);
        HIP_OK(hipMemcpyAsync(tm.data(), buf, tm.size() * 4, hipMemcpyDeviceToHost, s));
        HIP_OK(hipStreamSynchronize(s));
        tap->resize(tm.size());
        for (size_t r = 0; r < rows; r++) for (int ch = 0; ch < C; ch++) (*tap)[(size_t) ch * rows + r] = tm[r * (size_t) C + ch];
    };
    grab(0, Bf, D, (size_t) Ts);
    int tmul = 1;
    float * pcm_dev = nullptr;
    auto tail = [&](bool taps) {
        launch_add(s, R, Bf, (size_t) D * Ts, A);
        if (taps) grab(1, A, D, (size_t) Ts);
        launch_act_round(s, A, (size_t) D * Ts, 1, H0);
        tmul = 1;
        for (int b = 0; b < 4; b++) {
            const CodecModel::Block & bl = cm.blocks[b];
            ConvTmArgs u = conv_args(bl.up.wm, bl.up.w32, bl.up.b, bl.up.cin, bl.up.cout, bl.up.k, bl.up.stride, H0, tmul);
// ... 807 lines not shown
```

bark.cpp_amd/csrc/engine_internal.h:

```cpp
#pragma once
#include "engine.h"

#include <algorithm>
#include <chrono>
#include <cstdlib>
#include <functional>
#include <stdexcept>
#include <string>
#include <vector>

#define HIP_OK(expr)                                                                                         \
    do {                                                                                                     \
        hipError_t _e = (expr);                                                                              \
        if (_e != hipSuccess)                                                                                \
            throw std::runtime_error(std::string("HIP error: ") + hipGetErrorString(_e) + " at " #expr);   \
    } while (0)

#ifdef BARK_TRACE
#define BARK_TRACE_SET(c, args, nwaves) do { (args).tr.rec = (c)->trace_rec; (args).tr.pos = (c)->trace_pos; (args).tr.cap = (c)->trace_cap; (args).tr.kid = (c)->trace_kid++; (args).tr.base = (c)->trace_base; (args).tr.per_replay = (c)->trace_per_replay; (c)->trace_base += (unsigned) (nwaves); } while (0)
#else
#define BARK_TRACE_SET(c, args, nwaves) do { } while (0)
#endif

namespace barkhip { namespace detail {
// ... 26 lines not shown
    }
    HIP_OK(hipMalloc(&p, bytes));
    ctx->allocs.push_back(p);
    if (poison_allocations() && ctx->stream) {
        HIP_OK(hipMemsetAsync(p, 0xFF, bytes, ctx->stream));
        HIP_OK(hipStreamSynchronize(ctx->stream));
    }
    return (T *) p;
}
int guard_check(bark_context * ctx, const char * where);
template <typename T> T * host_alloc(bark_context * ctx, size_t count) {
    void * p = nullptr;
    HIP_OK(hipHostMalloc(&p, std::max<size_t>(count, 1) * sizeof(T), hipHostMallocDefault));
    ctx->pinned.push_back(p);
    return (T *) p;
}
} }

template <typename T> void barkhip::DevBuf<T>::reserve(bark_context * ctx, size_t count) {
    if (count > n) { p = detail::dev_alloc<T>(ctx, count); n = count; }
}
inline void barkhip::Event::record(hipStream_t s) {
    if (!e) HIP_OK(hipEventCreate(&e));
    HIP_OK(hipEventRecord(e, s));
}

namespace barkhip { namespace detail {

inline void copy_to_host(bark_context * c, void * dst, const void * src, size_t bytes) {
    HIP_OK(hipMemcpyAsync(dst, src, bytes, hipMemcpyDeviceToHost, c->stream));
    HIP_OK(hipStreamSynchronize(c->stream));
}

inline QMat q4_rows(const QMat & w, size_t row0, int K) {
    QMat r = w;
    if (w.qt == QT_F32) { r.qs = w.qs + row0 * (size_t) K * 4; return r; }
    const size_t nb = row0 * (size_t) (K / 32);
    r.d = w.d + nb; r.qs = w.qs + nb * (size_t) quant_formats()[w.qt].qs_bytes;
    if (w.m) r.m = w.m + nb;
    if (w.qh) r.qh = w.qh + nb;
    return r;
}

double weight_bytes_per_element(const GptModel & m);
inline GptRun & run_of(bark_context * c, const GptModel & m) { return c->gpt_run[&m - c->gpt]; }
inline float * layer_k(bark_context * c, const GptModel & m, int l) { return run_of(c, m).kcache + m.kv_layer_stride * (size_t) l; }
inline float * layer_v(bark_context * c, const GptModel & m, int l) { return run_of(c, m).vcache + m.kv_layer_stride * (size_t) l; }
inline float * layer_vt(bark_context * c, const GptModel & m, int l) { float * vt = run_of(c, m).vtcache; return vt ? vt + m.kv_layer_stride * (size_t) l : nullptr; }
struct RowBufs { float * x, * q; half_t * xn, * att, * hbuf, * q16, * k16, * vt16; float * logits; const int32_t * tokens; int plane; };
RowBufs own_rows(bark_context * c);
bool fine_products_on_f16_mfma(const bark_context * c, const GptModel & m, bool causal);
struct JobScope {
    bark_context * c; bool prev;
    explicit JobScope(bark_context * ctx) : c(ctx), prev(ctx->in_job) { ctx->in_job = true; }
    ~JobScope() { c->in_job = prev; }
    JobScope(const JobScope &) = delete; JobScope & operator=(const JobScope &) = delete;
};
enum LayerOp { OP_QKV = 0, OP_PROJ = 1, OP_FC = 2, OP_MPROJ = 3 };
LinArgs layer_product(const bark_context * c, const GptModel & m, int l, int op);
LinArgs lm_head_args(const GptModel & m, int row0, int n_rows, int parity_rows, const float * xrow, float * out, int ld_out, const StepState * st);
template <typename Args> void set_token_embedding(Args & a, const bark_context * c, const GptModel & m) {
    a.wte = m.wte[0]; a.wte_q = m.wte_q[0]; a.wpe = m.wpe; a.E = m.hp.n_embd; a.n_in = m.hp.n_in_vocab; a.P = c->P;
}
void embed_state_row(bark_context * c, const GptModel & m, const StepState * st, float * x);
GraphExec capture_graph(hipStream_t s, const std::function<void()> & body);
double time_on_stream_us(bark_context * c, const std::function<void()> & body);
void run_layers_rows(bark_context * c, GptModel & m, int N, bool causal, float * kbase = nullptr, float * vbase = nullptr, int pos0 = 0,
                     const RowBufs * rb = nullptr, int seq = 0, size_t kv_seq_stride = 0, const SeqTab * seqtab = nullptr);
void run_layers_decode(bark_context * c, GptModel & m);
void run_lm_head(bark_context * c, GptModel & m, const float * xrow, int row0, int n_rows, int parity_rows, float out_div = 0.0f);
void set_state(bark_context * c, const StepState & st);
StepState get_state(bark_context * c);
StepState fresh_state();
void upload_tokens(bark_context * c, const int32_t * tok, size_t n);
void check_ids(const int32_t * tok, size_t n, int n_in, const char * what);
int run_prefill(bark_context * c, GptModel & m, int n_tokens, bool merge, float * kbase = nullptr, float * vbase = nullptr, int pos0 = 0);
struct StageCfg {
    int which; int mode; int lm_row0, lm_rows, parity_rows; int token_base; float min_eos_p; int eos_token; float temp;
};
StageCfg stage_cfg(bark_context * c, int which);
void run_sample(bark_context * c, const StageCfg & s, int n_past_add, bool prescaled = false);
void enqueue_decode_step(bark_context * c, const StageCfg & s, bool sample, int n_past_add, bool embed = true);
GraphExec capture_decode(bark_context * c, const StageCfg & s, int n_past_add, int n_steps = 1, int ng = 4);
void decode_steps_greedy(bark_context * c, const StageCfg & s, int n, int n_past);
int sample_host(std::vector<float> & l, std::mt19937 & rng, float temp, float * eos_p, const bark_hip_sampling_filter * flt = nullptr);
void filter_host(std::vector<float> & l, int32_t top_k, float top_p);
std::vector<float> fetch_logits(bark_context * c, size_t n);
void upload_uniforms(bark_context * c, int n);
void upload_filter(bark_context * c);
void consume_uniforms(bark_context * c, int n_used);
void progress(bark_context * c, bark_encoding_step step, int pct);
void run_fine_forward(bark_context * c, int nn, int n_rows, const RowBufs * rb = nullptr, int Z = 1);
struct FinePlan { int T = 0, L = 0, n_loops = 0, n_hist = 0; std::vector<int32_t> in_arr; };
struct FineWindow { int start_idx, start_fill_idx, rel; };
FinePlan fine_plan(const bark_context_params & p, const std::vector<int32_t> & coarse, const VoicePrompt * voice = nullptr);
std::vector<int32_t> fine_plan_result(FinePlan & f);
FineWindow fine_window(const FinePlan & f, int n);
struct VoiceTrim { std::vector<int32_t> sem, coarse; };
VoiceTrim voice_trim(const bark_context_params & p, const VoicePrompt * v);
std::vector<int32_t> coarse_window_prompt(const bark_context_params & p, const VoiceTrim & vt, const std::vector<int32_t> & semantic, const std::vector<int32_t> & out, int step_idx);
void fine_window_tokens(const FinePlan & f, const FineWindow & w, int32_t * tok, size_t plane);
void fine_write_back(FinePlan & f, const FineWindow & w, const bark_context_params & p, const int32_t * tok, size_t plane);
void ensure_fine_batch(bark_context * c, int Z);
RowBufs fine_batch_rows(bark_context * c, int Z);

} }
```

bark.cpp_amd/csrc/engine_load.hip:

```cpp
#include "engine_internal.h"

#include <algorithm>
#include <climits>
#include <cmath>
#include <cstdio>
#include <cstdlib>
#include <cstring>
#include <deque>
#include <stdexcept>

using namespace barkhip;
using namespace barkhip::detail;

namespace {

struct SlabPlan {
    struct Item { const uint8_t * src; size_t bytes; size_t off; };
    std::vector<Item> items;
    size_t total = 0;
    size_t add(const TensorRef & t) {
        const size_t off = total;
        items.push_back({t.data, t.nbytes(), off});
        total = (total + t.nbytes() + 255) & ~(size_t) 255;
        return off;
// ... 62 lines not shown
int guard_check(bark_context * ctx, const char * where) {
    if (ctx->guarded.empty() || !ctx->stream) return 0;
    int bad = 0;
    std::vector<unsigned char> h(kGuardBytes);
    HIP_OK(hipStreamSynchronize(ctx->stream));
    for (size_t i = 0; i < ctx->guarded.size(); i++) {
        for (int side = 0; side < 2; side++) {
            const char * g = (const char *) ctx->guarded[i].first + (side ? kGuardBytes + ctx->guarded[i].second : 0);
            HIP_OK(hipMemcpyAsync(h.data(), g, kGuardBytes, hipMemcpyDeviceToHost, ctx->stream));
            HIP_OK(hipStreamSynchronize(ctx->stream));
            size_t first = kGuardBytes, n = 0;
            for (size_t k = 0; k < kGuardBytes; k++) if (h[k] != 0xA5) { if (first == kGuardBytes) first = k; n++; }
            if (n) {
                bad++;
                fprintf(stderr, "bark-hip GUARD DAMAGED (%s, ctx %p): allocation %zu (%zu bytes), %s band: %zu bytes overwritten, first at offset %zu (value 0x%02x)\n",
                        where, (void *) ctx, i, ctx->guarded[i].second, side ? "upper" : "lower", n, first, h[first]);
                HIP_OK(hipMemsetAsync((void *) g, 0xA5, kGuardBytes, ctx->stream));
            }
        }
    }
    HIP_OK(hipStreamSynchronize(ctx->stream));
    return bad;
}
}

void engine_invalidate_graphs(bark_context * ctx) {
    if (ctx->tail) engine_invalidate_graphs(ctx->tail);
    ctx->batch_graphs.clear();
    for (auto & g : ctx->fine_graphs) g.reset();
    for (auto & r : ctx->gpt_run) {
        for (auto & e : r.decode_graph) e.reset();
        for (auto & e : r.decode_graph8) e.reset();
        r.bench_graph.reset();
    }
}

static void init_runtime(bark_context * ctxp, bool weights_uploaded_now) {
    struct Holder { bark_context * p; bark_context * get() const { return p; } bark_context * operator->() const { return p; } } ctx{ctxp};
    const int P = ctx->P;
    for (int g = 0; g < 2; g++) {
        const GptModel & m = ctx->gpt[g];
        GptRun & r = ctx->gpt_run[g];
        r.kcache = dev_alloc<float>(ctx.get(), m.kv_layer_stride * m.hp.n_layer);
        r.vcache = dev_alloc<float>(ctx.get(), m.kv_layer_stride * m.hp.n_layer);
        r.vtcache = dev_alloc<float>(ctx.get(), m.kv_layer_stride * m.hp.n_layer);
    }
    {
        const GptModel & m = ctx->gpt[2];
        GptRun & r = ctx->gpt_run[2];
        r.kcache = dev_alloc<float>(ctx.get(), (size_t) m.hp.n_embd * P);
        r.vcache = dev_alloc<float>(ctx.get(), (size_t) m.hp.n_embd * P);
    }
    const size_t NE = (size_t) P * ctx->max_E;
    ctx->x = dev_alloc<float>(ctx.get(), NE);
    ctx->q = dev_alloc<float>(ctx.get(), NE);
    ctx->xn = dev_alloc<half_t>(ctx.get(), NE);
    ctx->att = dev_alloc<half_t>(ctx.get(), NE);
    ctx->hbuf = dev_alloc<half_t>(ctx.get(), NE * 4);
    if (ctx->fast_gemm) {
        ctx->q16 = dev_alloc<half_t>(ctx.get(), NE);
        ctx->k16 = dev_alloc<half_t>(ctx.get(), NE);
        ctx->vt16 = dev_alloc<half_t>(ctx.get(), NE);
    }
    ctx->ps = dev_alloc<float>(ctx.get(), (size_t) ctx->max_H * P * 4);
    ctx->knew = dev_alloc<float>(ctx.get(), (size_t) ctx->max_E);
    HIP_OK(hipMemsetAsync(ctx->ps, 0, (size_t) ctx->max_H * P * 4 * sizeof(float), ctx->stream));
    if (ctx->any_q4) {
        ctx->att32 = dev_alloc<float>(ctx.get(), NE);
        ctx->h32 = dev_alloc<float>(ctx.get(), NE * 4);
        const size_t nT = (size_t) (4 * ctx->max_E / 32) * 1024;
        ctx->xq.q = dev_alloc<int8_t>(ctx.get(), NE * 4);
        ctx->xq.d = dev_alloc<float>(ctx.get(), NE * 4 / 32);
        ctx->xq.s = dev_alloc<float>(ctx.get(), NE * 4 / 32);
        ctx->xq.dT = dev_alloc<float>(ctx.get(), nT);
        ctx->xq.sT = dev_alloc<float>(ctx.get(), nT);
        HIP_OK(hipMemsetAsync(ctx->xq.dT, 0, nT * sizeof(float), ctx->stream));
        HIP_OK(hipMemsetAsync(ctx->xq.sT, 0, nT * sizeof(float), ctx->stream));
        if (ctx->any_w32) ctx->xn32 = dev_alloc<float>(ctx.get(), NE);
    }
    size_t n_logits = (size_t) 1024 * ctx->gpt[2].hp.n_out_vocab;
    for (int g = 0; g < 2; g++) n_logits = std::max(n_logits, (size_t) ctx->gpt[g].hp.n_out_vocab);
    ctx->logits = dev_alloc<float>(ctx.get(), n_logits);
    ctx->d_tokens = dev_alloc<int32_t>(ctx.get(), 8 * 1024);
    ctx->d_out_tokens = dev_alloc<int32_t>(ctx.get(), 2048);
    ctx->d_eos_trace = dev_alloc<float>(ctx.get(), 2048);
    ctx->d_state = dev_alloc<StepState>(ctx.get(), 1);
    ctx->d_lstm_t = dev_alloc<int>(ctx.get(), 2);
    ctx->d_u = dev_alloc<double>(ctx.get(), 8192);
    ctx->d_filter = dev_alloc<int32_t>(ctx.get(), 2);
    ctx->d_fine_rel = dev_alloc<int32_t>(ctx.get(), 1);
    HIP_OK(hipMemsetAsync(ctx->d_fine_rel, 0, 4, ctx->stream));
    { const char * e = getenv("BARK_HIP_HOST_SAMPLING"); ctx->host_sampling = e && atoi(e) != 0; }
    {
        std::vector<uint16_t> lut(65536);
        for (uint32_t i = 0; i < 65536; i++) {
            const uint16_t bits = (uint16_t) i;
            const _Float16 h = __builtin_bit_cast(_Float16, bits);
            const _Float16 r = (_Float16) gelu_tanh_host((float) h);
            lut[i] = __builtin_bit_cast(uint16_t, r);
        }
        ctx->d_gelu_lut = dev_alloc<uint16_t>(ctx.get(), 65536);
        HIP_OK(hipMemcpyAsync(ctx->d_gelu_lut, lut.data(), 65536 * 2, hipMemcpyHostToDevice, ctx->stream));
        HIP_OK(hipStreamSynchronize(ctx->stream));
    }
    HIP_OK(hipStreamSynchronize(ctx->stream));
    if (weights_uploaded_now) HIP_OK(hipDeviceSynchronize());
}

bark_context * engine_load(const char * path, const bark_context_params & params, uint32_t seed, int device) {
    int n_dev = 0;
    if (hipGetDeviceCount(&n_dev) != hipSuccess || n_dev <= 0)
        throw std::runtime_error("no HIP device available (this engine has no CPU path)");
    std::unique_ptr<bark_context> ctx(new bark_context());
    ctx->params = params;
    ctx->rng = std::mt19937(seed);
    if (device >= 0) ctx->device = device;
    else if (const char * e = getenv("BARK_HIP_DEVICE")) ctx->device = atoi(e);
    else (void) hipGetDevice(&ctx->device);
    if (ctx->device < 0 || ctx->device >= n_dev) throw std::runtime_error("HIP device ordinal out of range (BARK_HIP_DEVICE / bark_hip_load_model_on_device)");
    HIP_OK(hipSetDevice(ctx->device));
    if (const char * e = getenv("BARK_HIP_GRAPH")) ctx->use_graph = atoi(e) != 0;
    if (const char * e = getenv("BARK_HIP_FAST_GEMM")) {
        if (!strcmp(e, "1")) ctx->fast_gemm = 1;
        else if (strcmp(e, "0") && *e) throw std::runtime_error("BARK_HIP_FAST_GEMM accepts 0 or 1");
    }
    if (const char * e = getenv("BARK_HIP_FINE_ORDER")) {
        if (!strcmp(e, "c1")) ctx->fine_order = 1;
        else if (!strcmp(e, "c1m")) ctx->fine_order = 2;
        else if (*e) throw std::runtime_error("BARK_HIP_FINE_ORDER accepts c1 or c1m");
    }
    HIP_OK(hipStreamCreateWithFlags(&ctx->stream, hipStreamNonBlocking));
    init_kernel_attributes();

    ModelFile mf;
    std::string err;
    if (!mf.open(path, err)) throw std::runtime_error(std::string("failed to read '") + path + "': " + err);
    ctx->vocab.build(mf.vocab);

    SlabPlan plan;
    struct Fix { const void ** dst; size_t off; };
    std::vector<Fix> fixes;
    auto place = [&](const TensorRef & t, const void ** dst) { fixes.push_back({dst, plan.add(t)}); };
    struct Q4Job { const TensorRef * t; QMat * dst; };
    std::vector<Q4Job> q4_jobs;
    int n_w16 = 0, n_wq4 = 0, n_w32 = 0;
    GptModel * cur_model = nullptr;
    auto place_w = [&](const TensorRef & t, const half_t ** dst16, QMat * dstq) {
        if (quant_format_by_type(t.ttype)) { q4_jobs.push_back({&t, dstq}); n_wq4++; }
        else if (t.ttype == 0) { place(t, (const void **) &dstq->qs); dstq->qt = QT_F32; n_w32++; }
        else { place(t, (const void **) dst16); n_w16++; }
        (void) cur_model;
    };

    for (int g = 0; g < 3; g++) {
        GptModel & m = ctx->gpt[g];
        m.hp = mf.gpt[g].hp;
        const auto & T = mf.gpt[g].tensors;
        const int E = m.hp.n_embd;
        if (E / m.hp.n_head != 64) throw std::runtime_error("head_dim must be 64");
        if (E != 128 && E != 256 && E != 512 && E != 768 && E != 1024) throw std::runtime_error("n_embd must be one of 128, 256, 512, 768, 1024");
        if (m.hp.n_in_vocab <= 0 || m.hp.n_out_vocab <= 0 || m.hp.n_out_vocab > 12288) throw std::runtime_error("vocabulary sizes must be in 1..12288 (output) and positive (input)");
        if (m.hp.block_size != 1024) throw std::runtime_error("block_size must be 1024");
        if (m.hp.n_wtes > 8 || m.hp.n_lm_heads > 8 || m.hp.n_layer > 64) throw std::runtime_error("unsupported GPT shape");
        m.layers.resize((size_t) m.hp.n_layer);
        m.kv_layer_stride = g < 2 ? (size_t) E * ctx->P : 0;
        n_w16 = n_wq4 = n_w32 = 0;
        for (int i = 0; i < m.hp.n_wtes; i++) place_w(need_w(T, "model/wte/" + std::to_string(i), E, m.hp.n_in_vocab), &m.wte[i], &m.wte_q[i]);
        for (int i = 0; i < m.hp.n_lm_heads; i++) place_w(need_w(T, "model/lm_head/" + std::to_string(i), E, m.hp.n_out_vocab), &m.lm_head[i], &m.lm_head_q[i]);
        place(need(T, "model/wpe", 0, E, m.hp.block_size), (const void **) &m.wpe);
// ... 425 lines not shown
```

bark.cpp_amd/csrc/kernels.h:

```cpp
#pragma once
#include "quant_formats.h"

#include <hip/hip_runtime.h>
#include <cstdint>

namespace barkhip {

typedef _Float16 half_t;

[[noreturn]] void kernel_fail(const char * fmt, ...) __attribute__((format(printf, 1, 2)));

struct StepState {
    int32_t n_past;
    int32_t cur_token;
    int32_t step;
    int32_t eos_step;
    int32_t near_tie;
    int32_t n_out;
    float   last_eos_p;
    int32_t fault;
};

struct QMat {
    const half_t * d = nullptr; const uint8_t * qs = nullptr; const half_t * m = nullptr; const uint32_t * qh = nullptr;
    int qt = 0;
};
struct Q8Scratch { int8_t * q = nullptr; float * d = nullptr, * dT = nullptr, * s = nullptr, * sT = nullptr; };

#ifdef BARK_TRACE
struct TraceSink { unsigned long long * rec = nullptr; unsigned * pos = nullptr; unsigned cap = 0; int kid = 0; unsigned base = 0, per_replay = 0; };
#define BARK_TRACE_FIELD TraceSink tr;
#else
#define BARK_TRACE_FIELD
#endif

struct SeqTab { int slot, pos0, len, pad; };

enum LinEpi { EPI_QKV = 0, EPI_RESID = 1, EPI_GELU = 2, EPI_LOGITS = 3, EPI_QKV16 = 4 };

struct LinArgs {
    const half_t * W = nullptr; int M = 0, K = 0;
    int N = 1;
    const half_t * x_f16 = nullptr;
    const float * x_f32 = nullptr; const float * ln_g = nullptr; const float * ln_b = nullptr;
    const float * ln_stats = nullptr;
    QMat wq;
    Q8Scratch xq;
    const float * bias = nullptr;
    int epi = EPI_LOGITS;
    float * q = nullptr; float * kc = nullptr; float * vc = nullptr; int E = 0, P = 0; int pos0 = 0;
    float * vt = nullptr;
    const StepState * st = nullptr;
    float * res = nullptr;
    half_t * out_h = nullptr; const uint16_t * lut = nullptr;
    float * out_h32 = nullptr;
    float * out = nullptr; int ld_out = 0;
    float * ps = nullptr; int ng = 4;
    float * knew = nullptr;
    float out_div = 0.0f;
    int parity_rows = 0;
    int batched = 0, nbatch = 1; size_t kv_slot_stride = 0;
    int fast = 0;
    half_t * q16 = nullptr, * k16 = nullptr, * vt16 = nullptr; int seq = 0;
    const SeqTab * seqtab = nullptr;
    BARK_TRACE_FIELD
};
void launch_linear(hipStream_t s, const LinArgs & a);
void launch_linear_slots(hipStream_t s, const LinArgs & a);
bool linear_slots_fuses_ln(int K);
void launch_linear_slots_ps(hipStream_t s, const LinArgs & a);
void launch_linear_slots_gemv(hipStream_t s, const LinArgs & a);

struct EmbedArgs {
    const half_t * wte = nullptr; const float * wpe = nullptr; int E = 0, n_in = 0, P = 1024;
    QMat wte_q;
    const int32_t * tokens = nullptr;
    int n_rows = 1; int merge = 0;
    int pos0 = 0;
    const StepState * st = nullptr;
    float * x = nullptr;
};
void launch_embed_causal(hipStream_t s, const EmbedArgs & a);
void launch_embed_fine(hipStream_t s, const half_t * const wte[8], const QMat * wte_q, const float * wpe, int E, int n_in,
                       const int32_t * tokens, int nn, float * x, int n_rows = 1024, int plane = 1024);

void launch_ln_stats(hipStream_t s, const float * x, int N, int E, float * stats);
void launch_q8_rows(hipStream_t s, const float * x, int N, int K, const float * ln_g, const float * ln_b, const Q8Scratch & out);
void launch_ln_rows(hipStream_t s, const float * x, int N, int E, const float * g, const float * b, half_t * out);
void launch_ln_rows_f32(hipStream_t s, const float * x, int N, int E, const float * g, const float * b, float * out);

struct AttnDecodeArgs {
    const float * q = nullptr; const float * kc = nullptr; const float * vc = nullptr;
    int H = 0, P = 0; const StepState * st = nullptr; half_t * att = nullptr;
    float * att32 = nullptr;
    const float * vt = nullptr;
    int ng = 4;
    const float * knew = nullptr;
    const float * ps = nullptr;
    int nbatch = 1; size_t kv_slot_stride = 0;
    float * sc = nullptr;
    BARK_TRACE_FIELD
};
void launch_attn_decode(hipStream_t s, const AttnDecodeArgs & a);

struct AttnPrefillArgs {
    const float * q = nullptr; int ldq = 0; const float * kc = nullptr; const float * vc = nullptr;
    int H = 0, P = 0, N = 0, n_past = 0; int causal = 1;
    half_t * att = nullptr; int ld_att = 0;
    float * att32 = nullptr;
    int Z = 1; size_t kv_seq_stride = 0;
    const SeqTab * seqtab = nullptr;
};
void launch_attn_prefill(hipStream_t s, const AttnPrefillArgs & a);
struct AttnFlashArgs {
    const half_t * q16 = nullptr, * k16 = nullptr, * vt16 = nullptr;
    int H = 0, E = 0, S = 0, Z = 1;
    half_t * att = nullptr; int ld_att = 0;
};
void launch_attn_flash(hipStream_t s, const AttnFlashArgs & a);
void launch_linear_fast(hipStream_t s, const LinArgs & a);
void init_fast_attributes();

struct SampleArgs {
    const float * logits = nullptr; int n = 0;
    int mode = 0;
    float temp = 0.0f;
    const double * u = nullptr;
    int u_stride = 0;
    float min_eos_p = 0.2f; int eos_token = 10000;
    int prescaled = 0;
    int force_exact = 0;
    int token_base = 0;
    int n_past_add = 1;
    int32_t * out_tokens = nullptr; float * eos_trace = nullptr; StepState * st = nullptr;
    int nbatch = 1; int ld_logits = 0; int out_stride = 0;
    const float * slot_temp = nullptr; const float * slot_min_eos_p = nullptr; int kinds = 0;
    const half_t * wte = nullptr; const float * wpe = nullptr; int E = 0, n_in = 0, P = 1024; float * x = nullptr;
    QMat wte_q;
    BARK_TRACE_FIELD
};
void launch_sample_greedy(hipStream_t s, const SampleArgs & a);
struct FilterArgs {
    float * logits = nullptr; int n = 0; int ld_logits = 0; int nbatch = 1;
    float temp = 0.0f; const float * slot_temp = nullptr;
    const int32_t * top_k = nullptr; const float * top_p = nullptr;
};
void launch_sample_filter(hipStream_t s, const FilterArgs & f);
void launch_sample_filtered(hipStream_t s, const SampleArgs & a, const int32_t * top_k, const float * top_p);
void launch_sample_rows_multinomial(hipStream_t s, const float * logits, int ld, int n_rows, int n_cols, float temp, const double * u,
                                    int32_t * out, int out_stride, StepState * st = nullptr, const int32_t * rel = nullptr);
void launch_argmax_rows(hipStream_t s, const float * logits, int ld, int n_rows, int n_cols, int32_t * out,
                        int out_stride, StepState * st, const int32_t * rel = nullptr);

int crosscheck_mask();
int exact_sampling();
int xcd_panel_width(int n_tiles, int ncol);
void init_kernel_attributes();
void init_attention_attributes();
void init_quant_attributes();
void launch_linear_q(hipStream_t s, const LinArgs & a);
void launch_linear_w32(hipStream_t s, const LinArgs & a);

struct CodecBatch { const int * T = nullptr; const int * Tpre = nullptr; int B = 1; };
void launch_rvq_gather(hipStream_t s, const float * codebooks, int n_bins, int Hd, const int32_t * codes, int n_q, int T, int rows_total, float * z, const CodecBatch & cb);
void launch_act_round(hipStream_t s, const float * x, size_t n, int elu, half_t * out_h);
// ... 81 lines not shown
```

bark.cpp_amd/csrc/misc_kernels.hip:

```cpp
#include "device_utils.h"

#include <cfloat>
#include <cstdio>
#include <cstdlib>

namespace barkhip {

__global__ void embed_causal_kernel(const EmbedArgs a) {
    const int i = blockIdx.x;
    int tok, tok2 = -1, pos;
    if (a.st) { tok = a.st->cur_token; pos = min(a.st->n_past, a.P - 1); }
    else {
        pos = a.pos0 + i;
        if (a.merge) { if (i < 256) { tok = a.tokens[i]; tok2 = a.tokens[256 + i]; } else tok = a.tokens[512]; }
        else tok = a.tokens[i];
    }
    tok = min(max(tok, 0), a.n_in - 1);
    if (tok2 >= 0) tok2 = min(tok2, a.n_in - 1);
    const float * pe = a.wpe + (size_t) pos * a.E;
    float * out = a.x + (size_t) i * a.E;
    for (int e = threadIdx.x; e < a.E; e += blockDim.x) {
        float v = wte_elem(a.wte, a.wte_q, a.E, tok, e);
        if (tok2 >= 0) v = v + wte_elem(a.wte, a.wte_q, a.E, tok2, e);
        out[e] = v + pe[e];
    }
}
void launch_embed_causal(hipStream_t s, const EmbedArgs & a) {
    hipLaunchKernelGGL(embed_causal_kernel, dim3(a.n_rows), dim3(256), 0, s, a);
}

struct FineEmbedArgs { const half_t * wte[8]; QMat wte_q[8]; const float * wpe; int E, n_in; const int32_t * tok; int nn; float * x; int plane; };
__global__ void embed_fine_kernel(const FineEmbedArgs a) {
    const int i = blockIdx.x;
    float * out = a.x + (size_t) i * a.E;
    const float * pe = a.wpe + (size_t) (i & 1023) * a.E;
    for (int e = threadIdx.x; e < a.E; e += blockDim.x) {
        float v = 0.0f;
        for (int cb = 0; cb <= a.nn; cb++) {
            int id = a.tok[(size_t) cb * a.plane + i];
            id = min(max(id, 0), a.n_in - 1);
            v = v + wte_elem(a.wte[cb], a.wte_q[cb], a.E, id, e);
        }
        out[e] = v + pe[e];
    }
}
void launch_embed_fine(hipStream_t s, const half_t * const wte[8], const QMat * wte_q, const float * wpe, int E, int n_in,
                       const int32_t * tokens, int nn, float * x, int n_rows, int plane) {
    FineEmbedArgs a; for (int i = 0; i < 8; i++) { a.wte[i] = wte[i]; a.wte_q[i] = wte_q[i]; }
    a.wpe = wpe; a.E = E; a.n_in = n_in; a.tok = tokens; a.nn = nn; a.x = x; a.plane = plane;
    hipLaunchKernelGGL(embed_fine_kernel, dim3(n_rows), dim3(256), 0, s, a);
}

__global__ __launch_bounds__(256) void ln_rows_kernel(const float * x, int N, int E, const float * g, const float * b, half_t * out) {
    const int lane = threadIdx.x & 63;
    const int row = blockIdx.x * 4 + (threadIdx.x >> 6);
    if (row >= N) return;
    const float * xr = x + (size_t) row * E;
    double s1 = 0.0;
    for (int e = lane; e < E; e += 64) s1 += (double) xr[e];
    s1 = wave_sum(s1);
    const float mean = (float) (s1 / (double) E);
    double s2 = 0.0;
    for (int e = lane; e < E; e += 64) { const float v = xr[e] - mean; s2 += (double) (v * v); }
    s2 = wave_sum(s2);
    const float var = (float) (s2 / (double) E);
    const float scale = 1.0f / sqrtf(var + 1e-5f);
    half_t * o = out + (size_t) row * E;
    for (int e = lane; e < E; e += 64) {
        float v = (xr[e] - mean) * scale;
        v = v * g[e];
        if (b) v = v + b[e];
        o[e] = to_half(v);
    }
}
__global__ __launch_bounds__(256) void ln_stats_kernel(const float * x, int N, int E, float * stats) {
    const int lane = threadIdx.x & 63;
    const int row = blockIdx.x * 4 + (threadIdx.x >> 6);
    if (row >= N) return;
    const float * xr = x + (size_t) row * E;
    double s1 = 0.0;
    for (int e = lane; e < E; e += 64) s1 += (double) xr[e];
    s1 = wave_sum(s1);
    const float mean = (float) (s1 / (double) E);
    double s2 = 0.0;
    for (int e = lane; e < E; e += 64) { const float v = xr[e] - mean; s2 += (double) (v * v); }
    s2 = wave_sum(s2);
    const float var = (float) (s2 / (double) E);
    if (lane == 0) { stats[2 * row] = mean; stats[2 * row + 1] = 1.0f / sqrtf(var + 1e-5f); }
}
void launch_ln_stats(hipStream_t s, const float * x, int N, int E, float * stats) {
    hipLaunchKernelGGL(ln_stats_kernel, dim3((N + 3) / 4), dim3(256), 0, s, x, N, E, stats);
}
__global__ __launch_bounds__(256) void ln_rows_f32_kernel(const float * x, int N, int E, const float * g, const float * b, float * out) {
    const int lane = threadIdx.x & 63;
    const int row = blockIdx.x * 4 + (threadIdx.x >> 6);
    if (row >= N) return;
    const float * xr = x + (size_t) row * E;
    double s1 = 0.0;
    for (int e = lane; e < E; e += 64) s1 += (double) xr[e];
    s1 = wave_sum(s1);
    const float mean = (float) (s1 / (double) E);
    double s2 = 0.0;
    for (int e = lane; e < E; e += 64) { const float v = xr[e] - mean; s2 += (double) (v * v); }
    s2 = wave_sum(s2);
    const float var = (float) (s2 / (double) E);
    const float scale = 1.0f / sqrtf(var + 1e-5f);
    float * o = out + (size_t) row * E;
    for (int e = lane; e < E; e += 64) {
        float v = (xr[e] - mean) * scale;
        v = v * g[e];
        if (b) v = v + b[e];
// ... 653 lines not shown
```

include/bark_mi355x.h:

```cpp
#pragma once
#include "bark.h"

#ifdef __cplusplus
extern "C" {
#endif

enum bark_hip_model { BARK_HIP_SEMANTIC = 0, BARK_HIP_COARSE = 1, BARK_HIP_FINE = 2 };

BARK_API int bark_hip_hparams(struct bark_context * bctx, int which, int32_t * out10);

BARK_API void bark_hip_set_params(struct bark_context * bctx, struct bark_context_params params);

BARK_API int bark_hip_tokenize(struct bark_context * bctx, const char * text, int32_t * out513);
BARK_API int bark_hip_bert_tokenize(struct bark_context * bctx, const char * text, int32_t * out, int n_max);

BARK_API int bark_hip_gpt_eval(struct bark_context * bctx, int which, const int32_t * tokens, int n_tokens,
                               int n_past, int merge_ctx, float * logits);

BARK_API int bark_hip_fine_eval(struct bark_context * bctx, const int32_t * tokens_8x1024, int nn, float * logits);

BARK_API int bark_hip_semantic(struct bark_context * bctx, const int32_t * prompt513, int32_t * out, int capacity, float * eos_trace);
BARK_API int bark_hip_coarse(struct bark_context * bctx, const int32_t * semantic, int n_semantic, int32_t * out_Tx2, int capacity_rows);
BARK_API int bark_hip_fine(struct bark_context * bctx, const int32_t * coarse_Tx2, int T, int32_t * out_Tx8, int capacity_rows);
BARK_API int bark_hip_fine_many(struct bark_context * bctx, const int32_t * coarse_concat, const int * T, int n, int32_t * out_concat, int capacity_rows);
// ... 21 lines not shown
BARK_API int bark_hip_resample_24k_to_16k(struct bark_context * bctx, const float * pcm24k, int n, float * out16k, int capacity);
#define BARK_HIP_VOICE_AUDIO_MAX_SAMPLES 480000
BARK_API int bark_hip_voice_from_audio(struct bark_context * bctx, const float * pcm24k, int n_samples, int32_t * semantic, int semantic_capacity,
                                       int32_t * coarse_Tx2, int32_t * fine_Tx8, int capacity_rows, int32_t * n_semantic, int32_t * n_frames);
BARK_API int bark_hip_set_voice_from_audio(struct bark_context * bctx, const float * pcm24k, int n_samples);
BARK_API double bark_hip_time_resample(struct bark_context * bctx, int n, int iters);

enum bark_hip_sample_format { BARK_HIP_SAMPLE_F32 = 0, BARK_HIP_SAMPLE_S16 = 1, BARK_HIP_SAMPLE_MULAW = 2 };
struct bark_hip_audio_format { int32_t sample_rate; int32_t sample_format; };
BARK_API int bark_hip_resample_out_len(int n, int rate_in, int rate_out);
BARK_API int bark_hip_resample_table(int rate_in, int rate_out, float * out, int capacity, int32_t lmh[3]);
BARK_API int bark_hip_resample(struct bark_context * bctx, const float * pcm, int n, int rate_in, int rate_out, float * out, int capacity);
BARK_API int bark_hip_resample_many(struct bark_context * bctx, const float * const * pcm, const int * n, int count, int rate_in,
                                    const struct bark_hip_audio_format * to, void * out_concat, int capacity_bytes, int32_t * n_out);
BARK_API int bark_hip_get_audio_as(struct bark_context * bctx, const struct bark_hip_audio_format * fmt, void * out, int capacity_bytes);
BARK_API int bark_hip_batch_audio_as(struct bark_context * bctx, int i, const struct bark_hip_audio_format * fmt, void * out, int capacity_bytes);
BARK_API double bark_hip_time_resample_pair(struct bark_context * bctx, int n, int rate_in, int rate_out, int sample_format, int iters);

struct bark_hip_join_params {
    int32_t gap_samples;
    int32_t fade_samples;
    float   trim_threshold;
    int32_t trim_pad_frames;
};
struct bark_hip_long_params { int32_t max_tokens; int32_t chain; struct bark_hip_join_params join; };
BARK_API int bark_hip_split_text(struct bark_context * bctx, const char * text, int max_tokens, int32_t * spans_Nx2, int capacity_chunks);
BARK_API int bark_hip_generate_long(struct bark_context * bctx, const char * text, const struct bark_hip_long_params * long_params,
                                    const struct bark_hip_request_params * params, const struct bark_hip_sampling_filter * filter,
                                    const struct bark_hip_voice_prompt * voice);
BARK_API int bark_hip_long_audio_as(struct bark_context * bctx, const struct bark_hip_audio_format * fmt, void * out, int capacity_bytes);
BARK_API int bark_hip_long_chunks(struct bark_context * bctx, int32_t * out_Nx4, int capacity_chunks);
BARK_API int bark_hip_long_chunk_audio(struct bark_context * bctx, int i, float ** data);
BARK_API int bark_hip_long_chunk_tokens(struct bark_context * bctx, int i, int stage, int32_t * out, int capacity);
BARK_API int bark_hip_join_many(struct bark_context * bctx, const float * const * pcm, const int * n, int count, const struct bark_hip_join_params * params,
                                const struct bark_hip_audio_format * to, void * out, int capacity_bytes, int32_t * layout_Nx2);
BARK_API double bark_hip_time_join(struct bark_context * bctx, int count, int n_each, int rate_out, int sample_format, int iters);
BARK_API double bark_hip_time_join_activity(struct bark_context * bctx, int count, int n_each, int iters);

BARK_API int bark_hip_tempo_out_len(int n, int speed_permille);
BARK_API int bark_hip_tempo_window(float * out720);
BARK_API int bark_hip_tempo(struct bark_context * bctx, const float * pcm, int n, int speed_permille, float * out, int capacity);
BARK_API int bark_hip_tempo_many(struct bark_context * bctx, const float * const * pcm, const int * n, int count, const int32_t * speed_permille,
                                 const struct bark_hip_audio_format * to, void * out_concat, int capacity_bytes, int32_t * n_out);
BARK_API int bark_hip_tempo_positions(struct bark_context * bctx, const float * pcm, int n, int speed_permille, int32_t * pos, int capacity);
BARK_API int bark_hip_get_audio_at(struct bark_context * bctx, const struct bark_hip_audio_format * fmt, int speed_permille, void * out, int capacity_bytes);
BARK_API int bark_hip_batch_audio_at(struct bark_context * bctx, int i, const struct bark_hip_audio_format * fmt, int speed_permille, void * out, int capacity_bytes);
BARK_API int bark_hip_long_audio_at(struct bark_context * bctx, const struct bark_hip_audio_format * fmt, int speed_permille, void * out, int capacity_bytes);
BARK_API double bark_hip_time_tempo(struct bark_context * bctx, int count, int n_each, int speed_permille, int iters);

BARK_API struct bark_context * bark_hip_clone_context(struct bark_context * src, uint32_t seed);

BARK_API int bark_hip_generate_audio_batch(struct bark_context ** ctxs, const char * const * texts, int n);

BARK_API int bark_hip_generate_batch(struct bark_context * bctx, const char * const * texts, int n);
BARK_API int bark_hip_generate_batch_seeded(struct bark_context * bctx, const char * const * texts, int n, const uint32_t * seeds);
struct bark_hip_request_params {
    float    temp;
    float    fine_temp;
    float    min_eos_p;
    int32_t  n_steps_text_encoder;
    uint32_t seed;
};
BARK_API int bark_hip_generate_batch_ex(struct bark_context * bctx, const char * const * texts, int n, const struct bark_hip_request_params * per_utterance);

struct bark_hip_sampling_filter {
    int32_t top_k;
    float   top_p;
};
BARK_API int bark_hip_set_sampling_filter(struct bark_context * bctx, int32_t top_k, float top_p);
BARK_API int bark_hip_generate_batch_filtered(struct bark_context * bctx, const char * const * texts, int n, const struct bark_hip_request_params * per_utterance,
                                              const struct bark_hip_sampling_filter * filters);
struct bark_hip_voice_prompt {
    const int32_t * semantic;   int32_t n_semantic;
    const int32_t * coarse_Tx2; int32_t n_coarse_frames;
    const int32_t * fine_Tx8;   int32_t n_fine_frames;
};
BARK_API int bark_hip_set_voice_prompt(struct bark_context * bctx, const struct bark_hip_voice_prompt * voice);
BARK_API int bark_hip_generate_batch_voiced(struct bark_context * bctx, const char * const * texts, int n, const struct bark_hip_request_params * per_utterance,
                                            const struct bark_hip_sampling_filter * filters, const struct bark_hip_voice_prompt * const * voices);
BARK_API int bark_hip_pick_rows(struct bark_context * bctx, const float * logits, int n_windows, int n_cols, float temp, const double * u,
                                const int32_t * rel, int32_t * tokens_io, int32_t * near_ties);
BARK_API int bark_hip_reserve_batch(struct bark_context * bctx, int slots);
BARK_API int bark_hip_batch_lock_steps(struct bark_context * bctx, int32_t out2[2]);
BARK_API int bark_hip_batch_audio(struct bark_context * bctx, int i, float ** data);
BARK_API int bark_hip_batch_tokens(struct bark_context * bctx, int i, int stage, int32_t * out, int capacity);

struct bark_hip_batcher;
BARK_API struct bark_hip_batcher * bark_hip_batcher_create(struct bark_context * bctx, int max_batch, int max_wait_ms);
BARK_API struct bark_hip_batcher * bark_hip_batcher_create_ex(struct bark_context * bctx, int max_batch, int max_wait_ms, int n_streams);
BARK_API struct bark_context * bark_hip_load_model_on_device(const char * model_path, struct bark_context_params params, uint32_t seed, int device);
BARK_API struct bark_hip_batcher * bark_hip_batcher_create_multi(struct bark_context * const * ctxs, int n_ctx, int max_batch, int max_wait_ms);
BARK_API int64_t bark_hip_batcher_submit(struct bark_hip_batcher * b, const char * text, uint32_t seed);
BARK_API int64_t bark_hip_batcher_submit_ex(struct bark_hip_batcher * b, const char * text, const struct bark_hip_request_params * params);
BARK_API int64_t bark_hip_batcher_submit_filtered(struct bark_hip_batcher * b, const char * text, const struct bark_hip_request_params * params,
                                                  const struct bark_hip_sampling_filter * filter);
BARK_API int64_t bark_hip_batcher_submit_voiced(struct bark_hip_batcher * b, const char * text, const struct bark_hip_request_params * params,
                                                const struct bark_hip_sampling_filter * filter, const struct bark_hip_voice_prompt * voice);
BARK_API int bark_hip_batcher_wait(struct bark_hip_batcher * b, int64_t ticket, float * pcm, int capacity);
BARK_API int64_t bark_hip_batcher_submit_as(struct bark_hip_batcher * b, const char * text, const struct bark_hip_request_params * params,
                                            const struct bark_hip_sampling_filter * filter, const struct bark_hip_voice_prompt * voice,
                                            const struct bark_hip_audio_format * fmt);
BARK_API int bark_hip_batcher_wait_bytes(struct bark_hip_batcher * b, int64_t ticket, void * out, int capacity_bytes);
BARK_API int64_t bark_hip_batcher_submit_long(struct bark_hip_batcher * b, const char * text, const struct bark_hip_long_params * long_params,
                                              const struct bark_hip_request_params * params, const struct bark_hip_sampling_filter * filter,
                                              const struct bark_hip_voice_prompt * voice, const struct bark_hip_audio_format * fmt);
BARK_API int bark_hip_batcher_ticket_chunks(struct bark_hip_batcher * b, int64_t ticket);
BARK_API int64_t bark_hip_batcher_submit_at(struct bark_hip_batcher * b, const char * text, const struct bark_hip_request_params * params,
                                            const struct bark_hip_sampling_filter * filter, const struct bark_hip_voice_prompt * voice,
                                            const struct bark_hip_audio_format * fmt, int speed_permille);
BARK_API int64_t bark_hip_batcher_submit_long_at(struct bark_hip_batcher * b, const char * text, const struct bark_hip_long_params * long_params,
                                                 const struct bark_hip_request_params * params, const struct bark_hip_sampling_filter * filter,
                                                 const struct bark_hip_voice_prompt * voice, const struct bark_hip_audio_format * fmt, int speed_permille);
BARK_API void bark_hip_batcher_stats(struct bark_hip_batcher * b, int * n_batches, int * n_requests, int * largest_batch);
BARK_API int bark_hip_batcher_admitted(struct bark_hip_batcher * b);
BARK_API void bark_hip_batcher_free(struct bark_hip_batcher * b);

BARK_API int bark_hip_get_semantic_tokens(struct bark_context * bctx, int32_t * out, int capacity);
BARK_API int bark_hip_get_coarse_tokens(struct bark_context * bctx, int32_t * out_Tx2, int capacity_rows);
BARK_API int bark_hip_get_fine_tokens(struct bark_context * bctx, int32_t * out_Tx8, int capacity_rows);

struct bark_hip_stats {
    int64_t t_load_us, t_eval_us;
    int64_t t_semantic_us, t_coarse_us, t_fine_us, t_codec_us;
    int64_t n_sample_semantic, n_sample_coarse, n_sample_fine;
    int32_t n_semantic, n_frames, n_samples;
    int32_t n_near_tie;
    int32_t graph_replays;
    int32_t n_prefix_rows_reused;
};
BARK_API void bark_hip_get_stats(struct bark_context * bctx, struct bark_hip_stats * out);

BARK_API double bark_hip_time_decode_step(struct bark_context * bctx, int which, int ctx, int iters,
                                          double * bytes_per_step);

BARK_API double bark_hip_time_gemv(struct bark_context * bctx, int which, int op, int iters, double * bytes_per_launch);

BARK_API double bark_hip_time_slots(struct bark_context * bctx, int which, int op, int n_slots, int kind, int ctx, int iters);

BARK_API int bark_hip_profile_lock_step(struct bark_context * bctx, int which, int n_slots, int ctx, int reps, char * json_out, int capacity);

BARK_API int bark_hip_sample_rows_filtered(struct bark_context * bctx, const float * logits, int n_rows, int n, const float * temp, const int32_t * top_k,
                                           const float * top_p, const double * u, int32_t * out_ids, float * out_eos_p);
BARK_API double bark_hip_time_sample_filter(struct bark_context * bctx, int n, int n_slots, int32_t top_k, float top_p, int peaked, int iters);

BARK_API double bark_hip_time_fine_pass(struct bark_context * bctx, int iters, double * flops_per_pass);
BARK_API double bark_hip_time_fine_passes(struct bark_context * bctx, int n_windows, int iters, double * flops_per_pass);

BARK_API int bark_hip_set_fine_order(struct bark_context * bctx, int order);
BARK_API const char * bark_hip_describe(struct bark_context * bctx);

#ifdef __cplusplus
}
#endif
```

Measured before the change: 23.25 audio-s/s.

## Queue semantic and coarse stages on device, removing per-upload host syncs

```diff
diff --git a/bark.cpp_amd/api.py b/bark.cpp_amd/api.py
--- a/bark.cpp_amd/api.py
+++ b/bark.cpp_amd/api.py
@@ -115,7 +115,7 @@
     "bark_hip_has_codec_encoder", "bark_hip_codec_encode", "bark_hip_codec_encode_many", "bark_hip_codec_encode_tap", "bark_hip_rvq_encode", "bark_hip_codec_encode_latents", "bark_hip_codec_encode_device_us",
     "bark_hip_load_semantic_encoder", "bark_hip_has_semantic_encoder", "bark_hip_semantic_encode", "bark_hip_semantic_encode_tap", "bark_hip_semantic_head", "bark_hip_semantic_encode_device_us",
     "bark_hip_resample_taps", "bark_hip_resample_24k_to_16k", "bark_hip_voice_from_audio", "bark_hip_set_voice_from_audio", "bark_hip_time_resample",
-    "bark_hip_batch_lock_steps",
+    "bark_hip_batch_lock_steps", "bark_hip_coarse_plan",
     "bark_hip_resample_out_len", "bark_hip_resample_table", "bark_hip_resample", "bark_hip_resample_many", "bark_hip_get_audio_as", "bark_hip_batch_audio_as",
     "bark_hip_batcher_submit_as", "bark_hip_batcher_wait_bytes", "bark_hip_time_resample_pair",
     "bark_hip_split_text", "bark_hip_generate_long", "bark_hip_long_audio_as", "bark_hip_long_chunks", "bark_hip_long_chunk_audio", "bark_hip_long_chunk_tokens",
@@ -240,6 +240,9 @@
     lib.bark_hip_batch_tokens.argtypes = [vp, C.c_int, C.c_int, ip, C.c_int]
     lib.bark_hip_batch_lock_steps.restype = C.c_int
     lib.bark_hip_batch_lock_steps.argtypes = [vp, C.POINTER(C.c_int32)]
+    if hasattr(lib, "bark_hip_coarse_plan"):
+        lib.bark_hip_coarse_plan.restype = C.c_int
+        lib.bark_hip_coarse_plan.argtypes = [C.POINTER(BarkContextParams), C.c_int, C.c_int, C.c_int, C.c_int, C.c_int, C.POINTER(C.c_int32), C.c_int]
     lib.bark_hip_clone_context.restype = vp
     lib.bark_hip_clone_context.argtypes = [vp, C.c_uint32]
     lib.bark_hip_generate_audio_batch.argtypes = [C.POINTER(C.c_void_p), C.POINTER(C.c_char_p), C.c_int]
diff --git a/bark.cpp_amd/csrc/api.hip b/bark.cpp_amd/csrc/api.hip
--- a/bark.cpp_amd/csrc/api.hip
+++ b/bark.cpp_amd/csrc/api.hip
@@ -1,4 +1,5 @@
 #include "engine.h"
+#include "engine_internal.h"
 
 #include <algorithm>
 #include <chrono>
@@ -830,6 +831,22 @@
     return 0;
 }
 
+int bark_hip_coarse_plan(const struct bark_context_params * params, int block_size, int n_semantic, int n_voice_semantic, int n_voice_coarse, int n_steps,
+                         int32_t * out_Wx6, int capacity_windows) {
+    if (!params || n_semantic < 0 || n_voice_semantic < 0 || n_voice_coarse < 0) return -1;
+    try {
+        const detail::CoarsePlan plan = detail::coarse_plan(*params, block_size, n_semantic, n_voice_semantic, n_voice_coarse, n_steps, true);
+        const int W = (int) plan.windows.size();
+        if (!out_Wx6 || capacity_windows < W) return -2;
+        for (int w = 0; w < W; w++) {
+            const detail::CoarseWindow & f = plan.windows[(size_t) w];
+            const int32_t row[6] = {f.N, f.L, f.steps_here, f.lay.sem_start, f.lay.hist_start, f.ng};
+            memcpy(out_Wx6 + (size_t) w * 6, row, sizeof(row));
+        }
+        return W;
+    } catch (...) { return -1; }
+}
+
 static int copy_out(const std::vector<int32_t> & v, int per_row, int32_t * out, int capacity_rows) {
     const int rows = (int) v.size() / per_row;
     if (!out || capacity_rows < rows) return -1;
diff --git a/bark.cpp_amd/csrc/engine.h b/bark.cpp_amd/csrc/engine.h
--- a/bark.cpp_amd/csrc/engine.h
+++ b/bark.cpp_amd/csrc/engine.h
@@ -39,6 +39,8 @@
 private:
     hipEvent_t e = nullptr;
 };
+constexpr int kStageOutCap = 16384;
+constexpr int kStageSlots = 4, kStageSlotBytes = 32 * 1024;
 template <typename T> struct DevBuf {
     T * p = nullptr; size_t n = 0;
     void reserve(bark_context * ctx, size_t count);
@@ -154,6 +156,10 @@
     int32_t * d_tokens = nullptr, * d_out_tokens = nullptr;
     float * d_eos_trace = nullptr;
     barkhip::StepState * d_state = nullptr;
+    barkhip::DevBuf<int32_t> d_stage_ids;
+    std::vector<barkhip::Event> stage_ev;
+    barkhip::StepState * h_poll = nullptr;
+    struct Staging { uint8_t * base = nullptr; barkhip::Event done[barkhip::kStageSlots]; bool busy[barkhip::kStageSlots] = {}; int next = 0; } staging;
     double * d_u = nullptr;
     bool host_sampling = false;
     bark_hip_sampling_filter filter{0, 1.0f};
diff --git a/bark.cpp_amd/csrc/engine.hip b/bark.cpp_amd/csrc/engine.hip
--- a/bark.cpp_amd/csrc/engine.hip
+++ b/bark.cpp_amd/csrc/engine.hip
@@ -157,10 +157,24 @@
     launch_linear(c->stream, a);
 }
 
-void set_state(bark_context * c, const StepState & st) {
-    HIP_OK(hipMemcpyAsync(c->d_state, &st, sizeof(st), hipMemcpyHostToDevice, c->stream));
-    HIP_OK(hipStreamSynchronize(c->stream));
-}
+void stage_upload(bark_context * c, void * dst, const void * src, size_t bytes) {
+    if (bytes == 0) return;
+    if (bytes > (size_t) kStageSlotBytes || host_driven_stages()) {
+        HIP_OK(hipMemcpyAsync(dst, src, bytes, hipMemcpyHostToDevice, c->stream));
+        HIP_OK(hipStreamSynchronize(c->stream));
+        return;
+    }
+    bark_context::Staging & r = c->staging;
+    const int i = r.next;
+    if (r.busy[i]) { HIP_OK(hipEventSynchronize(r.done[i].get())); r.busy[i] = false; }
+    uint8_t * slot = r.base + (size_t) i * kStageSlotBytes;
+    memcpy(slot, src, bytes);
+    HIP_OK(hipMemcpyAsync(dst, slot, bytes, hipMemcpyHostToDevice, c->stream));
+    r.done[i].record(c->stream);
+    r.busy[i] = true;
+    r.next = (i + 1) % kStageSlots;
+}
+void set_state(bark_context * c, const StepState & st) { stage_upload(c, c->d_state, &st, sizeof(st)); }
 StepState get_state(bark_context * c) {
     StepState st;
     HIP_OK(hipMemcpyAsync(&st, c->d_state, sizeof(st), hipMemcpyDeviceToHost, c->stream));
@@ -174,10 +188,7 @@
     return st;
 }
 
-void upload_tokens(bark_context * c, const int32_t * tok, size_t n) {
-    HIP_OK(hipMemcpyAsync(c->d_tokens, tok, n * 4, hipMemcpyHostToDevice, c->stream));
-    HIP_OK(hipStreamSynchronize(c->stream));
-}
+void upload_tokens(bark_context * c, const int32_t * tok, size_t n) { stage_upload(c, c->d_tokens, tok, n * 4); }
 
 void check_ids(const int32_t * tok, size_t n, int n_in, const char * what) {
     for (size_t i = 0; i < n; i++)
@@ -270,11 +281,15 @@
     return capture_graph(c->stream, [&] { for (int i = 0; i < n_steps; i++) enqueue_decode_step(c, s, true, n_past_add, false); });
 }
 
-void decode_steps_greedy(bark_context * c, const StageCfg & s, int n, int n_past) {
+void decode_steps_greedy(bark_context * c, const StageCfg & s, int n, int n_past, const std::function<void(int)> * queued) {
     GptRun & run = c->gpt_run[s.which];
     if (!c->use_graph) {
         struct Restore { bark_context * c; ~Restore() { c->decode_ng = 4; } } restore{c};
-        for (int k = 0; k < n; k++) { c->decode_ng = std::min(4, (n_past + k + 256) / 256); enqueue_decode_step(c, s, true, 1, false); }
+        for (int k = 0; k < n; k++) {
+            c->decode_ng = std::min(4, (n_past + k + 256) / 256);
+            enqueue_decode_step(c, s, true, 1, false);
+            if (queued) (*queued)(k + 1);
+        }
         return;
     }
     int k = 0;
@@ -286,6 +301,7 @@
         HIP_OK(hipGraphLaunch(e.get(), c->stream));
         c->stats.graph_replays++;
         k += g;
+        if (queued) (*queued)(k);
     }
 }
 
@@ -367,8 +383,7 @@
 void upload_filter(bark_context * c) {
     int32_t v[2] = {c->filter.top_k, 0};
     memcpy(&v[1], &c->filter.top_p, 4);
-    HIP_OK(hipMemcpyAsync(c->d_filter, v, sizeof(v), hipMemcpyHostToDevice, c->stream));
-    HIP_OK(hipStreamSynchronize(c->stream));
+    stage_upload(c, c->d_filter, v, sizeof(v));
 }
 
 void progress(bark_context * c, bark_encoding_step step, int pct) {
@@ -541,12 +556,36 @@
         progress(c, SEMANTIC, 100 * 1 / std::max(1, p.n_steps_text_encoder));
         int issued = 1;
         StepState cur{};
-        while (true) {
-            const int batch_end = std::min(n_steps, issued + 32);
-            decode_steps_greedy(c, s, batch_end - issued, N + issued - 1);
-            for (; issued < batch_end; issued++) progress(c, SEMANTIC, 100 * (issued + 1) / std::max(1, p.n_steps_text_encoder));
-            cur = get_state(c);
-            if (cur.eos_step != INT32_MAX || issued >= n_steps) break;
+        if (host_driven_stages()) {
+            while (true) {
+                const int batch_end = std::min(n_steps, issued + 32);
+                decode_steps_greedy(c, s, batch_end - issued, N + issued - 1);
+                for (; issued < batch_end; issued++) progress(c, SEMANTIC, 100 * (issued + 1) / std::max(1, p.n_steps_text_encoder));
+                cur = get_state(c);
+                if (cur.eos_step != INT32_MAX || issued >= n_steps) break;
+            }
+        } else {
+            DrainOnThrow drain(c);
+            if (c->stage_ev.size() < 2) c->stage_ev.resize(2);
+            int queued = 1;
+            auto queue_batch = [&](int k) {
+                const int end = std::min(n_steps, queued + 32);
+                decode_steps_greedy(c, s, end - queued, N + queued - 1);
+                launch_state_snapshot(c->stream, c->d_state, &c->h_poll[k & 1]);
+                c->stage_ev[(size_t) (k & 1)].record(c->stream);
+                queued = end;
+                return end;
+            };
+            int end_k = queue_batch(0);
+            for (int k = 0; ; k++) {
+                const int end_next = end_k < n_steps ? queue_batch(k + 1) : end_k;
+                HIP_OK(hipEventSynchronize(c->stage_ev[(size_t) (k & 1)].get()));
+                cur = c->h_poll[k & 1];
+                if (cur.fault) throw std::runtime_error("decode step launched with a context bound below the cached keys (partial scores incomplete)");
+                for (; issued < end_k; issued++) progress(c, SEMANTIC, 100 * (issued + 1) / std::max(1, p.n_steps_text_encoder));
+                if (cur.eos_step != INT32_MAX || issued >= n_steps) break;
+                end_k = end_next;
+            }
         }
         const int n_keep = std::min(cur.eos_step, issued);
         out.resize((size_t) n_keep);
@@ -596,19 +635,127 @@
     for (int k = n_flat - n_ch; k < n_flat - 2; k++) t.coarse.push_back(p.semantic_vocab_size + p.codebook_size * (k % nc) + v->coarse[(size_t) k]);
     return t;
 }
-std::vector<int32_t> coarse_window_prompt(const bark_context_params & p, const VoiceTrim & vt, const std::vector<int32_t> & semantic, const std::vector<int32_t> & out, int step_idx) {
+CoarseLayout coarse_window_layout(const bark_context_params & p, int n_sh, int n_semantic, int n_vc, int step_idx, int n_generated) {
     const float stc_ratio = p.coarse_rate_hz / p.semantic_rate_hz * p.n_coarse_codebooks;
     const int max_semantic_history = (int) floorf(p.max_coarse_history / stc_ratio);
-    const int n_sh = (int) vt.sem.size(), n_all = n_sh + (int) semantic.size();
+    const int n_all = n_sh + n_semantic;
     const int semantic_idx = n_sh + (int) roundf(step_idx / stc_ratio);
+    CoarseLayout l;
+    l.sem_start = std::max(semantic_idx - max_semantic_history, 0);
+    l.sem_count = std::max(0, std::min(256, n_all - l.sem_start));
+    const int total = n_vc + n_generated;
+    l.hist_count = std::min(p.max_coarse_history, total);
+    l.hist_start = total - l.hist_count;
+    return l;
+}
+std::vector<int32_t> coarse_window_prompt(const bark_context_params & p, const VoiceTrim & vt, const std::vector<int32_t> & semantic, const std::vector<int32_t> & out, int step_idx) {
+    const int n_sh = (int) vt.sem.size(), n_vc = (int) vt.coarse.size();
+    const CoarseLayout l = coarse_window_layout(p, n_sh, (int) semantic.size(), n_vc, step_idx, (int) out.size());
     std::vector<int32_t> in;
     in.reserve(257 + (size_t) p.max_coarse_history);
-    for (int i = std::max(semantic_idx - max_semantic_history, 0); i < n_all && in.size() < 256; i++) in.push_back(i < n_sh ? vt.sem[(size_t) i] : semantic[(size_t) (i - n_sh)]);
+    for (int i = l.sem_start; i < l.sem_start + l.sem_count; i++) in.push_back(i < n_sh ? vt.sem[(size_t) i] : semantic[(size_t) (i - n_sh)]);
     in.resize(256, p.coarse_semantic_pad_token);
     in.push_back(p.coarse_infer_token);
-    const int n_vc = (int) vt.coarse.size(), total = n_vc + (int) out.size();
-    for (int k = total - std::min(p.max_coarse_history, total); k < total; k++) in.push_back(k < n_vc ? vt.coarse[(size_t) k] : out[(size_t) (k - n_vc)]);
+    for (int k = l.hist_start; k < l.hist_start + l.hist_count; k++) in.push_back(k < n_vc ? vt.coarse[(size_t) k] : out[(size_t) (k - n_vc)]);
     return in;
+}
+CoarsePlan coarse_plan(const bark_context_params & p, int block_size, int n_semantic, int n_sh, int n_vc, int n_steps, bool reuse_prefix) {
+    if (p.sliding_window_size <= 0 || p.max_coarse_history < 0) throw std::runtime_error("coarse: bad window parameters");
+    if (n_steps <= 0) throw std::runtime_error("coarse: no steps to run");
+    constexpr int32_t kPad = -1, kInfer = -2, kHist = 1 << 28;
+    CoarsePlan plan;
+    plan.n_steps = n_steps;
+    const int n_windows = (int) ceilf((float) n_steps / p.sliding_window_size);
+    std::vector<int32_t> cached, in;
+    int step_idx = 0;
+    for (int w = 0; w < n_windows; w++) {
+        CoarseWindow f;
+        f.lay = coarse_window_layout(p, n_sh, n_semantic, n_vc, step_idx, step_idx);
+        in.clear();
+        for (int i = 0; i < 256; i++) in.push_back(i < f.lay.sem_count ? f.lay.sem_start + i : kPad);
+        in.push_back(kInfer);
+        for (int k = 0; k < f.lay.hist_count; k++) in.push_back(kHist + f.lay.hist_start + k);
+        f.step_idx = step_idx;
+        f.N = (int) in.size();
+        f.steps_here = std::min(p.sliding_window_size, n_steps - step_idx);
+        if (f.N + f.steps_here - 1 > block_size)
+            throw std::runtime_error(w == 0 && n_vc > 0 ? "coarse: the voice prompt's history and the first window exceed the context" : "coarse: window exceeds the context");
+        f.L = 0;
+        if (reuse_prefix) {
+            while (f.L < f.N && f.L < (int) cached.size() && cached[(size_t) f.L] == in[(size_t) f.L]) f.L++;
+            if (f.L >= f.N) f.L = f.N - 1;
+        }
+        f.ng = std::min(4, (f.N + f.steps_here - 1 + 255) / 256);
+        plan.windows.push_back(f);
+        cached = in;
+        for (int j = 0; j + 1 < f.steps_here; j++) cached.push_back(kHist + n_vc + step_idx + j);
+        step_idx += f.steps_here;
+    }
+    return plan;
+}
+
+std::vector<int32_t> coarse_stage_queued(bark_context * c, const StageCfg & s, const std::vector<int32_t> & semantic, const VoiceTrim & voice, int n_steps, bool reuse_prefix) {
+    const bark_context_params & p = c->params;
+    GptModel & m = c->gpt[1];
+    const int n_sh = (int) voice.sem.size(), n_vc = (int) voice.coarse.size(), n_sem = (int) semantic.size();
+    const CoarsePlan plan = coarse_plan(p, m.hp.block_size, n_sem, n_sh, n_vc, n_steps, reuse_prefix);
+    check_ids(voice.sem.data(), voice.sem.size(), m.hp.n_in_vocab, "coarse");
+    check_ids(voice.coarse.data(), voice.coarse.size(), m.hp.n_in_vocab, "coarse");
+    const int32_t fixed[2] = {p.coarse_semantic_pad_token, p.coarse_infer_token};
+    check_ids(fixed, 2, m.hp.n_in_vocab, "coarse");
+    std::vector<int32_t> ids;
+    ids.reserve((size_t) (n_sh + n_sem + n_vc));
+    ids.insert(ids.end(), voice.sem.begin(), voice.sem.end());
+    ids.insert(ids.end(), semantic.begin(), semantic.end());
+    ids.insert(ids.end(), voice.coarse.begin(), voice.coarse.end());
+    c->d_stage_ids.reserve(c, ids.size());
+    DrainOnThrow drain(c);
+    stage_upload(c, c->d_stage_ids.p, ids.data(), ids.size() * 4);
+    set_state(c, fresh_state());
+    const size_t W = plan.windows.size();
+    const bool events = p.progress_callback != nullptr;
+    if (events && c->stage_ev.size() < W) c->stage_ev.resize(W);
+    size_t w = 0;
+    while (w < W) {
+        const CoarseWindow & f = plan.windows[w];
+        const int rows = f.N - f.L;
+        CoarsePromptArgs a;
+        a.sem = c->d_stage_ids.p; a.hist = c->d_stage_ids.p + n_sh + n_sem; a.out = c->d_out_tokens;
+        a.sem_start = f.lay.sem_start; a.sem_count = f.lay.sem_count; a.n_hist = n_vc; a.hist_start = f.lay.hist_start;
+        a.L = f.L; a.N = f.N; a.step = f.step_idx; a.pad_token = p.coarse_semantic_pad_token; a.infer_token = p.coarse_infer_token;
+        a.tokens = c->d_tokens; a.st = c->d_state;
+        if (rows < 2) throw std::runtime_error("coarse: a run of windows must start with a prompt pass");
+        launch_coarse_prompt(c->stream, a);
+        run_prefill(c, m, rows, false, nullptr, nullptr, f.L);
+        run_lm_head(c, m, c->x + (size_t) (rows - 1) * m.hp.n_embd, s.lm_row0, s.lm_rows, s.parity_rows);
+        run_sample(c, s, rows);
+        c->stats.n_prefix_rows_reused += f.L;
+        size_t e = w + 1;
+        while (e < W && plan.windows[e].N - plan.windows[e].L == 1) { c->stats.n_prefix_rows_reused += plan.windows[e].L; e++; }
+        const int chain = plan.windows[e - 1].step_idx + plan.windows[e - 1].steps_here - (f.step_idx + 1);
+        size_t v = w;
+        const std::function<void(int)> mark = [&](int k) {
+            while (v < e && plan.windows[v].step_idx + plan.windows[v].steps_here - (f.step_idx + 1) <= k) {
+                if (events) c->stage_ev[v].record(c->stream);
+                v++;
+            }
+        };
+        mark(0);
+        decode_steps_greedy(c, s, chain, f.N, &mark);
+        w = e;
+    }
+    if (events) {
+        for (size_t v = 0; v < W; v++) {
+            HIP_OK(hipEventSynchronize(c->stage_ev[v].get()));
+            for (int j = 0; j < plan.windows[v].steps_here; j++) progress(c, COARSE, 100 * (plan.windows[v].step_idx + j + 1) / n_steps);
+        }
+    }
+    std::vector<int32_t> out((size_t) n_steps);
+    HIP_OK(hipMemcpyAsync(out.data(), c->d_out_tokens, (size_t) n_steps * 4, hipMemcpyDeviceToHost, c->stream));
+    const StepState cur = get_state(c);
+    c->stats.n_sample_coarse += n_steps;
+    c->stats.n_near_tie += cur.near_tie;
+    return out;
 }
 }
 
@@ -658,7 +805,9 @@
     std::vector<int32_t> cached;
     const bool reuse_prefix = !(crosscheck_mask() & 8);
     int step_idx = 0;
-    for (int w = 0; w < n_windows; w++) {
+    const bool queued = greedy && !host_driven_stages() && n_steps <= kStageOutCap;
+    if (queued) out = coarse_stage_queued(c, s, semantic, voice, n_steps, reuse_prefix);
+    for (int w = 0; w < n_windows && !queued; w++) {
         const std::vector<int32_t> in = coarse_window_prompt(p, voice, semantic, out, step_idx);
         const int N = (int) in.size();
         const int steps_here = std::min(p.sliding_window_size, n_steps - step_idx);
@@ -748,7 +897,7 @@
         const FineWindow w = fine_window(plan, n);
         const int rel = w.rel;
         fine_window_tokens(plan, w, buf.data(), 1024);
-        HIP_OK(hipMemcpyAsync(c->d_fine_rel, &w.rel, 4, hipMemcpyHostToDevice, c->stream));
+        stage_upload(c, c->d_fine_rel, &w.rel, 4);
         upload_tokens(c, buf.data(), buf.size());
         if (device_multinomial) upload_uniforms(c, (nf - nc) * 1024);
         for (int nn = nc; nn < nf; nn++) {
diff --git a/bark.cpp_amd/csrc/engine_codec.hip b/bark.cpp_amd/csrc/engine_codec.hip
--- a/bark.cpp_amd/csrc/engine_codec.hip
+++ b/bark.cpp_amd/csrc/engine_codec.hip
@@ -50,8 +50,7 @@
         slot.out = out2; slot.gi = io.gi; slot.B = B;
     }
     const int hdr[2] = {0, Tmax};
-    HIP_OK(hipMemcpyAsync(c->d_lstm_t, hdr, sizeof(hdr), hipMemcpyHostToDevice, s));
-    HIP_OK(hipStreamSynchronize(s));
+    stage_upload(c, c->d_lstm_t, hdr, sizeof(hdr));
     for (int i0 = 0; i0 <= Tmax; i0 += kBlock) HIP_OK(hipGraphLaunch(slot.exec.get(), s));
 }
 
diff --git a/bark.cpp_amd/csrc/engine_internal.h b/bark.cpp_amd/csrc/engine_internal.h
--- a/bark.cpp_amd/csrc/engine_internal.h
+++ b/bark.cpp_amd/csrc/engine_internal.h
@@ -132,7 +132,7 @@
 void run_sample(bark_context * c, const StageCfg & s, int n_past_add, bool prescaled = false);
 void enqueue_decode_step(bark_context * c, const StageCfg & s, bool sample, int n_past_add, bool embed = true);
 GraphExec capture_decode(bark_context * c, const StageCfg & s, int n_past_add, int n_steps = 1, int ng = 4);
-void decode_steps_greedy(bark_context * c, const StageCfg & s, int n, int n_past);
+void decode_steps_greedy(bark_context * c, const StageCfg & s, int n, int n_past, const std::function<void(int)> * queued = nullptr);
 int sample_host(std::vector<float> & l, std::mt19937 & rng, float temp, float * eos_p, const bark_hip_sampling_filter * flt = nullptr);
 void filter_host(std::vector<float> & l, int32_t top_k, float top_p);
 std::vector<float> fetch_logits(bark_context * c, size_t n);
@@ -149,6 +149,19 @@
 struct VoiceTrim { std::vector<int32_t> sem, coarse; };
 VoiceTrim voice_trim(const bark_context_params & p, const VoicePrompt * v);
 std::vector<int32_t> coarse_window_prompt(const bark_context_params & p, const VoiceTrim & vt, const std::vector<int32_t> & semantic, const std::vector<int32_t> & out, int step_idx);
+struct CoarseLayout { int sem_start, sem_count, hist_start, hist_count; };
+CoarseLayout coarse_window_layout(const bark_context_params & p, int n_sh, int n_semantic, int n_vc, int step_idx, int n_generated);
+struct CoarseWindow { int step_idx, steps_here, N, L, ng; CoarseLayout lay; };
+struct CoarsePlan { int n_steps = 0; std::vector<CoarseWindow> windows; };
+CoarsePlan coarse_plan(const bark_context_params & p, int block_size, int n_semantic, int n_sh, int n_vc, int n_steps, bool reuse_prefix);
+void stage_upload(bark_context * c, void * dst, const void * src, size_t bytes);
+struct DrainOnThrow {
+    bark_context * c; int n;
+    explicit DrainOnThrow(bark_context * ctx) : c(ctx), n(std::uncaught_exceptions()) {}
+    ~DrainOnThrow() { if (std::uncaught_exceptions() > n) (void) hipStreamSynchronize(c->stream); }
+    DrainOnThrow(const DrainOnThrow &) = delete; DrainOnThrow & operator=(const DrainOnThrow &) = delete;
+};
+inline bool host_driven_stages() { return (crosscheck_mask() & 4096) != 0; }
 void fine_window_tokens(const FinePlan & f, const FineWindow & w, int32_t * tok, size_t plane);
 void fine_write_back(FinePlan & f, const FineWindow & w, const bark_context_params & p, const int32_t * tok, size_t plane);
 void ensure_fine_batch(bark_context * c, int Z);
diff --git a/bark.cpp_amd/csrc/engine_load.hip b/bark.cpp_amd/csrc/engine_load.hip
--- a/bark.cpp_amd/csrc/engine_load.hip
+++ b/bark.cpp_amd/csrc/engine_load.hip
@@ -168,9 +168,11 @@
     for (int g = 0; g < 2; g++) n_logits = std::max(n_logits, (size_t) ctx->gpt[g].hp.n_out_vocab);
     ctx->logits = dev_alloc<float>(ctx.get(), n_logits);
     ctx->d_tokens = dev_alloc<int32_t>(ctx.get(), 8 * 1024);
-    ctx->d_out_tokens = dev_alloc<int32_t>(ctx.get(), 2048);
+    ctx->d_out_tokens = dev_alloc<int32_t>(ctx.get(), kStageOutCap);
     ctx->d_eos_trace = dev_alloc<float>(ctx.get(), 2048);
     ctx->d_state = dev_alloc<StepState>(ctx.get(), 1);
+    ctx->h_poll = host_alloc<StepState>(ctx.get(), 2);
+    ctx->staging.base = host_alloc<uint8_t>(ctx.get(), (size_t) kStageSlots * kStageSlotBytes);
     ctx->d_lstm_t = dev_alloc<int>(ctx.get(), 2);
     ctx->d_u = dev_alloc<double>(ctx.get(), 8192);
     ctx->d_filter = dev_alloc<int32_t>(ctx.get(), 2);
diff --git a/bark.cpp_amd/csrc/kernels.h b/bark.cpp_amd/csrc/kernels.h
--- a/bark.cpp_amd/csrc/kernels.h
+++ b/bark.cpp_amd/csrc/kernels.h
@@ -81,6 +81,14 @@
     float * x = nullptr;
 };
 void launch_embed_causal(hipStream_t s, const EmbedArgs & a);
+struct CoarsePromptArgs {
+    const int32_t * sem = nullptr, * hist = nullptr, * out = nullptr;
+    int sem_start = 0, sem_count = 0, n_hist = 0, hist_start = 0;
+    int L = 0, N = 0, step = 0, pad_token = 0, infer_token = 0;
+    int32_t * tokens = nullptr; StepState * st = nullptr;
+};
+void launch_coarse_prompt(hipStream_t s, const CoarsePromptArgs & a);
+void launch_state_snapshot(hipStream_t s, const StepState * st, StepState * host_slot);
 void launch_embed_fine(hipStream_t s, const half_t * const wte[8], const QMat * wte_q, const float * wpe, int E, int n_in,
                        const int32_t * tokens, int nn, float * x, int n_rows = 1024, int plane = 1024);
 
diff --git a/bark.cpp_amd/csrc/misc_kernels.hip b/bark.cpp_amd/csrc/misc_kernels.hip
--- a/bark.cpp_amd/csrc/misc_kernels.hip
+++ b/bark.cpp_amd/csrc/misc_kernels.hip
@@ -27,6 +27,36 @@
 }
 void launch_embed_causal(hipStream_t s, const EmbedArgs & a) {
     hipLaunchKernelGGL(embed_causal_kernel, dim3(a.n_rows), dim3(256), 0, s, a);
+}
+
+__global__ __launch_bounds__(256) void coarse_prompt_kernel(const CoarsePromptArgs a) {
+    const int r = a.L + (int) (blockIdx.x * blockDim.x + threadIdx.x);
+    if (r >= a.N) return;
+    int id;
+    if (r < 256) id = r < a.sem_count ? a.sem[a.sem_start + r] : a.pad_token;
+    else if (r == 256) id = a.infer_token;
+    else {
+        const int k = a.hist_start + (r - 257);
+        id = k < a.n_hist ? a.hist[k] : a.out[k - a.n_hist];
+    }
+    a.tokens[r - a.L] = id;
+    if (r == a.L) { a.st->n_past = a.L; a.st->cur_token = id; a.st->step = a.step; }
+}
+void launch_coarse_prompt(hipStream_t s, const CoarsePromptArgs & a) {
+    if (a.N <= a.L || a.L < 0) kernel_fail("coarse prompt: no rows to build (L %d, N %d)", a.L, a.N);
+    hipLaunchKernelGGL(coarse_prompt_kernel, dim3((a.N - a.L + 255) / 256), dim3(256), 0, s, a);
+}
+
+__global__ void state_snapshot_kernel(const StepState * st, StepState * host_slot) {
+    if (threadIdx.x == 0 && blockIdx.x == 0) {
+        *host_slot = *st;
+#ifdef __HIP_DEVICE_COMPILE__
+        __threadfence_system();
+#endif
+    }
+}
+void launch_state_snapshot(hipStream_t s, const StepState * st, StepState * host_slot) {
+    hipLaunchKernelGGL(state_snapshot_kernel, dim3(1), dim3(64), 0, s, st, host_slot);
 }
 
 struct FineEmbedArgs { const half_t * wte[8]; QMat wte_q[8]; const float * wpe; int E, n_in; const int32_t * tok; int nn; float * x; int plane; };
diff --git a/include/bark_mi355x.h b/include/bark_mi355x.h
--- a/include/bark_mi355x.h
+++ b/include/bark_mi355x.h
@@ -127,6 +127,8 @@
                                 const int32_t * rel, int32_t * tokens_io, int32_t * near_ties);
 BARK_API int bark_hip_reserve_batch(struct bark_context * bctx, int slots);
 BARK_API int bark_hip_batch_lock_steps(struct bark_context * bctx, int32_t out2[2]);
+BARK_API int bark_hip_coarse_plan(const struct bark_context_params * params, int block_size, int n_semantic, int n_voice_semantic, int n_voice_coarse, int n_steps,
+                                  int32_t * out_Wx6, int capacity_windows);
 BARK_API int bark_hip_batch_audio(struct bark_context * bctx, int i, float ** data);
 BARK_API int bark_hip_batch_tokens(struct bark_context * bctx, int i, int stage, int32_t * out, int capacity);
 
```

After: 23.50 audio-s/s (median of 6 runs). 1.01x the previous value.
